# genetics-statistics/GEMMA

Hardware: AMD Instinct MI355X
Metric: SNPs/s (-lmm 1 Wald) at n=20k on 1/2/4/8 MI355X; U^T x HBM GB/s vs roofline (higher is better)
Workload: dtype f64 (U^T x as int8-digit MFMA products with exact int32 accumulation; every column of U scaled by its exact maximum and rounded to 6 base-256 digits = 2^-48 of that maximum -- fp64 keeps 2^-53 per entry; value_strict / strict_leg (7g6m: U^T x at or below the fp64 GEMM's own error) and fp64_gemm_path

## Files before the change

### gemma_amd/build.py

```python
import os
import shutil
import subprocess

HERE = os.path.dirname(os.path.abspath(__file__))
CSRC = os.path.join(HERE, "csrc")
LIB = os.path.join(HERE, "libgemma_hip.so")
UNITS = {
    "gemma_hip.hip": ["dgemm_mfma.hip.h", "lmm_grid.hip.h", "lmm_score_panel.hip.h", "i8gemm.hip.h", "i8gemm_sparse.hip.h", "i8gemm_sparse2.hip.h", "i8gemm_sparse2_r16.hip.h", "i8gemm_dense16.hip.h", "lmm_assoc.hip.h",
                      "lmm_search.hip.h", "comm.hip.h", "comm_shm.hpp", "kin_i8.hip.h", "ingest.hip.h", "qc.hip.h", "lm_assoc.hip.h", "mvlmm.hip.h",
                      "mvlmm_kernels.hip.h", "eigh_tu.h", "tu_common.h",
                      "abi_kinship.inc.h", "abi_eigen_qc.inc.h", "abi_lmm_stage.inc.h", "abi_utx.inc.h", "abi_lmm_batch.inc.h",
                      "abi_mvlmm.inc.h", "abi_gxe_lm.inc.h", "abi_kept_comm.inc.h", "abi_lmm_multi.inc.h", "abi_lmm_score_panel.inc.h", "abi_vc.inc.h", "vc_tu.h", "abi_prdt.inc.h", "prdt_tu.h",
                      "abi_mqs.inc.h", "mqs_tu.h", "abi_cor.inc.h", "cor_tu.h"],
    "eigh_tu.hip": ["dgemm_mfma.hip.h", "eigh.hip.h", "eigh2.hip.h", "eigh_tu.h", "tu_common.h"],
    "vc_tu.hip": ["dgemm_mfma.hip.h", "spd_inv.hip.h", "vc.hip.h", "vc_tu.h", "tu_common.h", "host_linalg.h", "../../include/gemma_vc_hybrid.hpp"],
    "prdt_tu.hip": ["dgemm_mfma.hip.h", "geno_mv.hip.h", "dev_common.hip.h", "eigh_tu.h", "prdt_tu.h", "tu_common.h", "spd_inv.hip.h", "prdt_mv.hip.h"],
    "mqs_tu.hip": ["dgemm_mfma.hip.h", "mqs.hip.h", "ci.hip.h", "dev_common.hip.h", "mqs_tu.h", "tu_common.h", "host_linalg.h"],
    "cor_tu.hip": ["dgemm_mfma.hip.h", "cor.hip.h", "dev_common.hip.h", "cor_tu.h", "tu_common.h"],
    "mvlmm_kernels.hip": ["mvlmm.hip.h", "mvlmm_kernels.hip.h"],
    "mvlmm_kernels_wide.hip": ["mvlmm.hip.h", "mvlmm_kernels.hip.h"],
    "mvlmm_kernels_rt.hip": ["mvlmm.hip.h", "mvlmm_kernels.hip.h"],
    "mvlmm_kernels_d6.hip": ["mvlmm.hip.h", "mvlmm_kernels.hip.h"],
    "mvlmm_kernels_d7.hip": ["mvlmm.hip.h", "mvlmm_kernels.hip.h"],
    "mvlmm_kernels_d8.hip": ["mvlmm.hip.h", "mvlmm_kernels.hip.h"],
}
PUBLIC_HEADER_USERS = ("gemma_hip.hip", "eigh_tu.hip", "vc_tu.hip", "prdt_tu.hip", "mqs_tu.hip", "cor_tu.hip")
SOURCES = list(UNITS)
HEADERS = sorted({h for hs in UNITS.values() for h in hs})


def hipcc():
    for cand in (os.environ.get("HIPCC"), "/opt/rocm/bin/hipcc", shutil.which("hipcc")):
        if cand and os.path.exists(cand):
            return cand
    raise RuntimeError("hipcc not found: the gfx950 library cannot be built")


def stale():
    if not os.path.exists(LIB):
        return True
    t = os.path.getmtime(LIB)
    deps = [os.path.join(CSRC, f) for f in SOURCES + HEADERS]
    deps.append(os.path.join(HERE, "..", "include", "gemma_hip.h"))
    return any(os.path.getmtime(d) > t for d in deps)


def build(force=False, verbose=False):
    if not force and not stale():
        return LIB
    cc = hipcc()
    objdir = os.path.join(HERE, "_obj")
    os.makedirs(objdir, exist_ok=True)
    procs, objs = [], []
    for src in SOURCES:
        obj = os.path.join(objdir, src.replace(".hip", ".o"))
        objs.append(obj)
        hdrs = UNITS[src]
        deps = [os.path.join(CSRC, f) for f in [src] + hdrs]
        if src in PUBLIC_HEADER_USERS:
            deps.append(os.path.join(HERE, "..", "include", "gemma_hip.h"))
        if not force and os.path.exists(obj) and all(os.path.getmtime(d) <= os.path.getmtime(obj) for d in deps):
            continue
        cmd = [cc, "--offload-arch=gfx950", "-O3", "-std=c++17", "-fPIC", "-c", os.path.join(CSRC, src), "-o", obj]
        if verbose:
            print(" ".join(cmd))
        procs.append((cmd, subprocess.Popen(cmd, cwd=CSRC)))
    for cmd, pr in procs:
        if pr.wait() != 0:
            raise subprocess.CalledProcessError(pr.returncode, cmd)
    cmd = [cc, "--offload-arch=gfx950", "-fPIC", "-shared", "-o", LIB] + objs
    if verbose:
        print(" ".join(cmd))
    subprocess.check_call(cmd, cwd=CSRC)
    return LIB


if __name__ == "__main__":
    print(build(force=True, verbose=True))
```

### gemma_amd/csrc/abi_lmm_batch.inc.h

```cpp

static void xp_release() {
  Ctx::XPipe &x = g_ctx.xp;
  if (x.P) (void)hipStreamDestroy(x.P);
  if (x.Q) (void)hipStreamDestroy(x.Q);
  if (x.in_ready) (void)hipEventDestroy(x.in_ready);
  if (x.ingest_done) (void)hipEventDestroy(x.ingest_done);
  x.ingest_done = nullptr;
  x.ingest_valid = false;
  for (int i = 0; i < 2; ++i) {
    if (x.prod_done[i]) (void)hipEventDestroy(x.prod_done[i]);
    if (x.post_done[i]) (void)hipEventDestroy(x.post_done[i]);
    x.prod_done[i] = x.post_done[i] = nullptr;
    x.post_valid[i] = false;
  }
  x.P = x.Q = nullptr;
  x.in_ready = nullptr;
  x.count = 0;
  x.pending = false;
  x.cus = -1;
  x.shadow_A.release(); x.shadow_C.release(); x.shadow_mean.release(); x.shadow_rowsur.release();
}
static int xp_init() {
  Ctx::XPipe &x = g_ctx.xp;
  const int ncu = g_ctx.prop.multiProcessorCount;
  int cus = g_ctx.knobs.pipe_cus;
  if (cus < 0 || cus * 2 > ncu || ncu % 32 != 0 || cus % 8 != 0 || (cus && (ncu / 8) % (cus / 8) != 0)) cus = 0;
  if (x.P && x.cus == cus) return GEMMA_HIP_OK;
  HIPCHK(hipDeviceSynchronize());
  xp_release();
  if (cus > 0) {
    const int words = ncu / 32, per_xcd = cus / 8, cu_per_xcd = ncu / 8, stepj = cu_per_xcd / per_xcd;
    std::vector<unsigned> mp((size_t)words, 0xFFFFFFFFu), mq((size_t)words, 0u);
    for (int j = 0; j < cu_per_xcd; j += stepj)
      for (int xcd = 0; xcd < 8; ++xcd) {
        const int c = 8 * j + xcd;
        mp[c >> 5] &= ~(1u << (c & 31));
        mq[c >> 5] |= 1u << (c & 31);
      }
    HIPCHK(hipExtStreamCreateWithCUMask(&x.P, (uint32_t)words, mp.data()));
    HIPCHK(hipExtStreamCreateWithCUMask(&x.Q, (uint32_t)words, mq.data()));
  } else {
    HIPCHK(hipStreamCreateWithFlags(&x.P, hipStreamDefault));
    HIPCHK(hipStreamCreateWithFlags(&x.Q, hipStreamDefault));
  }
  HIPCHK(hipEventCreateWithFlags(&x.in_ready, hipEventDisableTiming));
  HIPCHK(hipEventCreateWithFlags(&x.ingest_done, hipEventDisableTiming));
  for (int i = 0; i < 2; ++i) {
    HIPCHK(hipEventCreateWithFlags(&x.prod_done[i], hipEventDisableTiming));
    HIPCHK(hipEventCreateWithFlags(&x.post_done[i], hipEventDisableTiming));
  }
  x.cus = cus;
  return GEMMA_HIP_OK;
}
static int xp_flush(hipStream_t s) {
  Ctx::XPipe &x = g_ctx.xp;
  if (!x.pending) return GEMMA_HIP_OK;
  for (int i = 0; i < 2; ++i)
    if (x.post_valid[i]) HIPCHK(hipStreamWaitEvent(s, x.post_done[i], 0));
  x.pending = false;
  x.ingest_valid = false;
  return GEMMA_HIP_OK;
}
static int xp_abort(int rc) {
  Ctx::XPipe &x = g_ctx.xp;
  (void)hipDeviceSynchronize();
  x.count = 0;
  x.post_valid[0] = x.post_valid[1] = false;
  x.pending = false;
  x.ingest_valid = false;
  return rc;
}
static void xp_swap_sets() {
  Ctx::XPipe &x = g_ctx.xp;
  std::swap(g_ctx.i8_A, x.shadow_A); std::swap(g_ctx.i8_C, x.shadow_C);
  std::swap(g_ctx.i8_mean, x.shadow_mean); std::swap(g_ctx.i8_rowsur, x.shadow_rowsur);
}


static int compute_utx(int kind, const void *geno, size_t l, size_t ld, int path, double **UtX_out, size_t *ldx_out,
                       hipStream_t s) {
  {
    int rcf = xp_flush(s);
    if (rcf) return rcf;
  }
  const size_t n = g_ctx.cfg.n;
  const size_t ldx = (n + 1) & ~(size_t)1;
  const bool want_i8 = (path < 0 ? utx_i8_mode() == 1 : path == 1);
  const bool plink_i8 = want_i8 && kind == GEMMA_GENO_PLINK_2BIT;
  if (g_ctx.UtX.reserve(l * ldx * 8) || (!plink_i8 && g_ctx.X.reserve(l * ldx * 8)))
    return fail(GEMMA_HIP_ENOMEM, "lmm_batch: cannot allocate 2 x %zu bytes", l * ldx * 8);
  double *UtX = g_ctx.UtX.as<double>();
  *UtX_out = UtX;
  *ldx_out = ldx;
  g_ctx.last_utx_path = plink_i8 ? 1 : 0;
  if (plink_i8) return utx_plink_i8(geno, l, ld, UtX, ldx, s);
  double *X = g_ctx.X.as<double>();
  bool done = false;
  if (kind == GEMMA_GENO_F64_IDV_MAJOR) {
    {
      ProfScope ps(GEMMA_STAGE_INGEST, s);
      dim3 grid((unsigned)((l + 31) / 32), (unsigned)((n + 31) / 32));
      hipLaunchKernelGGL(transpose_kernel, grid, dim3(32, 8), 0, s, reinterpret_cast<const double *>(geno),
                         (long)n, (long)l, (long)ld, X, (long)ldx);
      HIPCHK(hipGetLastError());
    }
    if (want_i8) {
      int rc = utx_f64_try_i8(X, l, ldx, false, UtX, ldx, s, &done);
      if (rc) return rc;
    }
  } else if (kind == GEMMA_GENO_F64_SNP_MAJOR && want_i8) {
    int rc = utx_f64_try_i8(reinterpret_cast<const double *>(geno), l, ld, true, UtX, ldx, s, &done);
    if (rc) return rc;
  }
  if (done) return GEMMA_HIP_OK;
  if (kind != GEMMA_GENO_F64_IDV_MAJOR) {
    ProfScope ps(GEMMA_STAGE_INGEST, s);
    IngestArgs a;
    a.src = geno; a.ld = (long)ld; a.l = (long)l;
    a.idx_map = g_ctx.have_map ? g_ctx.idx_map.as<int>() : nullptr;
    a.n = (int)n; a.dst = X; a.ldo = (long)ldx; a.k_mode = 0;
    const unsigned grid = (unsigned)((l + 3) / 4);
    if (kind == GEMMA_GENO_PLINK_2BIT)
      hipLaunchKernelGGL(ingest_lmm_kernel<true>, dim3(grid), dim3(256), 0, s, a);
    else
      hipLaunchKernelGGL(ingest_lmm_kernel<false>, dim3(grid), dim3(256), 0, s, a);
    HIPCHK(hipGetLastError());
  }
  {
    ProfScope ps(GEMMA_STAGE_UTX_GEMM, s);
    const double *Ug;
    long ldu;
    int rcu = gemm_U(&Ug, &ldu, s);
    if (rcu) return rcu;
    note_utx_kernel(GEMMA_UTX_KERNEL_DGEMM_F64, 0, 0, 0);
    HIPCHK(launch_dgemm('N', 'N', (long)l, (long)n, (long)n, 1.0, X, (long)ldx, Ug, ldu, 0.0, UtX,
                        (long)ldx, false, false, s));
  }
  return GEMMA_HIP_OK;
}

static int check_batch_args(const char *who, int kind, const void *geno, size_t l, size_t ld, const void *out) {
  const size_t n = g_ctx.cfg.n;
  const size_t per_row = (kind == GEMMA_GENO_PLINK_2BIT && g_ctx.have_map) ? g_ctx.ni_total : n;
  const size_t need = min_ld_for(kind, per_row, l);
  if (need == (size_t)-1) return fail(GEMMA_HIP_EINVAL, "%s: unknown geno_kind %d", who, kind);
  if (!geno || !out || ld < need) return fail(GEMMA_HIP_EINVAL, "%s: ld=%zu < %zu", who, ld, need);
  return GEMMA_HIP_OK;
}

static int overlap_chunks(size_t l) {
  if (!g_ctx.knobs.overlap) return 1;
  if (utx_i8_mode() != 1 || i8_sparse_mode() != 2) return 1;
  int q = g_ctx.knobs.overlap_chunks;
  q = std::max(1, std::min(q, 16));
  while (q > 1 && l < (size_t)q * 2 * S2_BM) --q;
  return q;
}
static int overlap_init() {
  if (g_ctx.ov_stream) return GEMMA_HIP_OK;
  HIPCHK(hipStreamCreateWithFlags(&g_ctx.ov_stream, hipStreamNonBlocking));
  for (auto &e : g_ctx.ov_ready) HIPCHK(hipEventCreateWithFlags(&e, hipEventDisableTiming));
  HIPCHK(hipEventCreateWithFlags(&g_ctx.ov_done, hipEventDisableTiming));
  return GEMMA_HIP_OK;
}
static int lmm_batch_plink_chunked(const void *geno, size_t l, size_t ld, gemma_sumstat *out_d, int chunks, hipStream_t s) {
  const size_t n = g_ctx.cfg.n;
  const size_t ldx = (n + 1) & ~(size_t)1;
  int rc = overlap_init();
  if (rc) return rc;
  if (g_ctx.UtX.reserve(l * ldx * 8)) return fail(GEMMA_HIP_ENOMEM, "lmm_batch: cannot allocate %zu bytes", l * ldx * 8);
  double *UtX = g_ctx.UtX.as<double>();
  g_ctx.last_utx_path = 1;
  I8Dims d;
  if ((rc = i8_begin(l, &d, s))) return rc;
  {
    ProfScope ps(GEMMA_STAGE_INGEST, s);
    IngestI8Args a;
    a.src = reinterpret_cast<const unsigned char *>(geno); a.ld = (long)ld; a.l = (long)l;
    a.idx_map = g_ctx.have_map ? g_ctx.idx_map.as<int>() : nullptr;
    a.n = (int)d.n; a.A = g_ctx.i8_A.as<int8_t>(); a.ldk = (long)d.ldk;
    a.mean = g_ctx.i8_mean.as<double>();
    hipLaunchKernelGGL(ingest_i8_kernel, dim3((unsigned)((l + 3) / 4)), dim3(256), 0, s, a);
    HIPCHK(hipGetLastError());
  }
  if ((rc = i8_meta_build(d, s))) return rc;
  const size_t per = round_up((l + chunks - 1) / chunks, (size_t)S2_BM);
  hipStream_t side = g_ctx.ov_stream;
  int c = 0;
  for (size_t row0 = 0; row0 < l; row0 += per, ++c) {
    const size_t rows = std::min(per, l - row0), rows_pad = std::min(per, d.lpad - row0);
    if ((rc = i8_gemm_rows(d, row0, rows_pad, s, UtX, ldx, rows))) break;
    if (hipEventRecord(g_ctx.ov_ready[c], s) != hipSuccess || hipStreamWaitEvent(side, g_ctx.ov_ready[c], 0) != hipSuccess) {
      rc = fail(GEMMA_HIP_ERUNTIME, "lmm_batch: %s", hipGetErrorString(hipGetLastError()));
      break;
    }
    if ((rc = i8_post_rows(l, d, row0, rows, UtX, ldx, side))) break;
    if ((rc = launch_assoc(UtX + row0 * ldx, rows, ldx, out_d + row0, side))) break;
  }
  (void)hipEventRecord(g_ctx.ov_done, side);
  (void)hipStreamWaitEvent(s, g_ctx.ov_done, 0);
  return rc;
}

static int xp_flush_fwd(hipStream_t s) { return xp_flush(s); }

extern "C" int gemma_hip_lmm_pipe_flush(void *stream) {
  NEED_INIT();
  return xp_flush(S(stream));
}

extern "C" int gemma_hip_lmm_batch_pipe_d(int kind, const void *geno, size_t l, size_t ld, gemma_sumstat *out_d, void *stream) {
  NEED_INIT();
  if (!g_ctx.lmm_active) return fail(GEMMA_HIP_ESTATE, "lmm_batch_pipe before lmm_setup");
  NEED_SINGLE("lmm_batch_pipe");
  if (l == 0) return GEMMA_HIP_OK;
  int rc = check_batch_args("lmm_batch_pipe", kind, geno, l, ld, out_d);
  if (rc) return rc;
  hipStream_t s = S(stream);
  if (kind != GEMMA_GENO_PLINK_2BIT || utx_i8_mode() != 1 || i8_sparse_mode() != 2) {
    if ((rc = xp_flush(s))) return rc;
    return gemma_hip_lmm_batch_d(kind, geno, l, ld, out_d, stream);
  }
  if ((rc = xp_init())) return rc;
  Ctx::XPipe &x = g_ctx.xp;
  const int slot = (int)(x.count & 1);
  const size_t n = g_ctx.cfg.n;
  const size_t ldx = (n + 1) & ~(size_t)1;
  if (g_ctx.UtX.reserve(l * ldx * 8)) return fail(GEMMA_HIP_ENOMEM, "lmm_batch_pipe: cannot allocate %zu bytes", l * ldx * 8);
  if (s != nullptr && x.ingest_valid) HIPCHK(hipStreamWaitEvent(s, x.ingest_done, 0));
  xp_swap_sets();
  if (s != nullptr) {
    HIPCHK(hipEventRecord(x.in_ready, s));
    HIPCHK(hipStreamWaitEvent(x.P, x.in_ready, 0));
  }
  if (x.post_valid[slot]) HIPCHK(hipStreamWaitEvent(x.P, x.post_done[slot], 0));
  g_ctx.last_utx_path = 1;
  I8Dims d;
  if ((rc = i8_begin(l, &d, x.P, false))) return xp_abort(rc);
  {
    ProfScope ps(GEMMA_STAGE_INGEST, x.P);
    IngestI8Args a;
    a.src = reinterpret_cast<const unsigned char *>(geno); a.ld = (long)ld; a.l = (long)l;
    a.idx_map = g_ctx.have_map ? g_ctx.idx_map.as<int>() : nullptr;
    a.n = (int)d.n; a.A = g_ctx.i8_A.as<int8_t>(); a.ldk = (long)d.ldk;
    a.mean = g_ctx.i8_mean.as<double>();
    hipLaunchKernelGGL(ingest_i8_kernel, dim3((unsigned)((l + 3) / 4)), dim3(256), 0, x.P, a);
    if (hipGetLastError() != hipSuccess) return xp_abort(fail(GEMMA_HIP_ERUNTIME, "lmm_batch_pipe: ingest launch"));
  }
  if (hipEventRecord(x.ingest_done, x.P) != hipSuccess) return xp_abort(fail(GEMMA_HIP_ERUNTIME, "lmm_batch_pipe: event"));
  x.ingest_valid = true;
  if ((rc = i8_meta_build(d, x.P))) return xp_abort(rc);
  if ((rc = i8_gemm_rows(d, 0, d.lpad, x.P))) return xp_abort(rc);
  HIPCHK(hipEventRecord(x.prod_done[slot], x.P));
  HIPCHK(hipStreamWaitEvent(x.Q, x.prod_done[slot], 0));
  double *UtX = g_ctx.UtX.as<double>();
  rc = i8_post_rows(l, d, 0, l, UtX, ldx, x.Q);
  if (!rc) rc = launch_assoc(UtX, l, ldx, out_d, x.Q);
  (void)hipEventRecord(x.post_done[slot], x.Q);
  x.post_valid[slot] = true;
  x.pending = true;
  x.count += 1;
  return rc;
}

extern "C" int gemma_hip_lmm_batch_d(int kind, const void *geno, size_t l, size_t ld, gemma_sumstat *out_d,
                                     void *stream) {
  NEED_INIT();
  if (!g_ctx.lmm_active) return fail(GEMMA_HIP_ESTATE, "lmm_batch before lmm_setup");
  NEED_SINGLE("lmm_batch");
  if (l == 0) return GEMMA_HIP_OK;
  int rc = check_batch_args("lmm_batch", kind, geno, l, ld, out_d);
  if (rc) return rc;
  hipStream_t s = S(stream);
  if ((rc = xp_flush(s))) return rc;
  if (kind == GEMMA_GENO_PLINK_2BIT) {
    const int chunks = overlap_chunks(l);
    if (chunks > 1) return lmm_batch_plink_chunked(geno, l, ld, out_d, chunks, s);
  }
  double *UtX;
  size_t ldx;
  rc = compute_utx(kind, geno, l, ld, -1, &UtX, &ldx, s);
  if (rc) return rc;
  return launch_assoc(UtX, l, ldx, out_d, s);
}

extern "C" int gemma_hip_lmm_gene_batch_d(const double *Y_d, size_t l, size_t ld, gemma_sumstat *out_d, void *stream) {
  NEED_INIT();
  if (!g_ctx.lmm_active) return fail(GEMMA_HIP_ESTATE, "lmm_gene_batch before lmm_setup");
  NEED_SINGLE("lmm_gene_batch");
  if (l == 0) return GEMMA_HIP_OK;
  const size_t n = g_ctx.cfg.n, c = g_ctx.cfg.n_cvt;
  if (!Y_d || !out_d || ld < n) return fail(GEMMA_HIP_EINVAL, "lmm_gene_batch: ld=%zu < n=%zu", ld, n);
  hipStream_t s = S(stream);
  const size_t ldx = (n + 1) & ~(size_t)1;
  if (int rcf = xp_flush(S(stream))) return rcf;
  if (g_ctx.UtX.reserve(l * ldx * 8)) return fail(GEMMA_HIP_ENOMEM, "lmm_gene_batch: %zu bytes", l * ldx * 8);
  double *UtY = g_ctx.UtX.as<double>();
  {
    ProfScope ps(GEMMA_STAGE_UTX_GEMM, s);
    const double *Ug;
    long ldu;
    int rcu = gemm_U(&Ug, &ldu, s);
    if (rcu) return rcu;
    HIPCHK(launch_dgemm('N', 'N', (long)l, (long)n, (long)n, 1.0, Y_d, (long)ld, Ug, ldu, 0.0, UtY, (long)ldx,
                        false, false, s));
  }
  AssocArgs a = g_ctx.assoc_proto;
  a.UtX = UtY; a.ld = (long)ldx; a.l = (long)l;
  a.eval = g_ctx.eval; a.Uty = g_ctx.Uty; a.UtWt = g_ctx.UtWt.as<double>();
  a.out = reinterpret_cast<SumStat *>(out_d);
  a.grid_T = nullptr;
  a.have_grid = 0;
  const unsigned grid = (unsigned)((l + 3) / 4);
  {
    ProfScope ps(GEMMA_STAGE_ASSOC, s);
    switch (c) {
    case 1: hipLaunchKernelGGL(lmm_gene_kernel<1>, dim3(grid), dim3(256), 0, s, a); break;
    case 2: hipLaunchKernelGGL(lmm_gene_kernel<2>, dim3(grid), dim3(256), 0, s, a); break;
    case 3: hipLaunchKernelGGL(lmm_gene_kernel<3>, dim3(grid), dim3(256), 0, s, a); break;
    case 4: hipLaunchKernelGGL(lmm_gene_kernel<4>, dim3(grid), dim3(256), 0, s, a); break;
    default:
      if (c > (size_t)GEN_CMAX) {
        int rcw = wide_attr(lmm_gene_wide_kernel);
        if (rcw) return rcw;
        hipLaunchKernelGGL(lmm_gene_wide_kernel, dim3((unsigned)l), dim3(64), wide_lds_bytes(c), s, a, (int)c);
      } else {
        hipLaunchKernelGGL(lmm_gene_generic_kernel, dim3(grid), dim3(256), 0, s, a, (int)c);
      }
      break;
    }
    HIPCHK(hipGetLastError());
  }
  return GEMMA_HIP_OK;
}

extern "C" int gemma_hip_lmm_gene_batch(const double *Y, size_t l, size_t ld, gemma_sumstat *out) {
  NEED_INIT();
  if (!g_ctx.lmm_active) return fail(GEMMA_HIP_ESTATE, "lmm_gene_batch before lmm_setup");
  NEED_SINGLE("lmm_gene_batch");
  if (l == 0) return GEMMA_HIP_OK;
  const size_t n = g_ctx.cfg.n;
  if (!Y || !out || ld < n) return fail(GEMMA_HIP_EINVAL, "lmm_gene_batch: ld=%zu < n=%zu", ld, n);
  if (g_ctx.stage_in.reserve(l * ld * 8) || g_ctx.stage_out.reserve(l * sizeof(gemma_sumstat)))
    return fail(GEMMA_HIP_ENOMEM, "lmm_gene_batch: staging %zu bytes", l * ld * 8);
  HIPCHK(hipMemcpy(g_ctx.stage_in.p, Y, l * ld * 8, hipMemcpyHostToDevice));
  int rc = gemma_hip_lmm_gene_batch_d(g_ctx.stage_in.as<double>(), l, ld, g_ctx.stage_out.as<gemma_sumstat>(), nullptr);
  if (rc) return rc;
  HIPCHK(hipMemcpy(out, g_ctx.stage_out.p, l * sizeof(gemma_sumstat), hipMemcpyDeviceToHost));
  return GEMMA_HIP_OK;
}
```

### gemma_amd/csrc/abi_utx.inc.h

```cpp

struct I8Dims {
  size_t n, ldk, npad, lpad, mrows;
  int fuse, digits, nplanes;
  int mdrop;
  int complete;
  int epi;
};
static const int *i8_anymiss(const I8Dims &d) { return d.complete ? g_ctx.i8_rowsur.as<int>() + d.lpad : nullptr; }
static int i8_sparse_mode() { return g_ctx.knobs.i8_sparse; }
static int i8_begin(size_t l, I8Dims *d, hipStream_t s, bool allow_epi = true) {
  int rc = i8_prepare_u(s);
  if (rc) return rc;
  d->n = g_ctx.cfg.n; d->ldk = g_ctx.i8_ldk; d->npad = g_ctx.i8_npad;
  d->lpad = round_up(l, i8_sparse_mode() == 2 ? (size_t)S2_BM : (size_t)I8P_BM); d->mrows = 2 * d->lpad;
  d->fuse = (g_ctx.knobs.i8_fuse && (double)d->n * 2.0 * 128.0 * 257.0 < 2147483648.0) ? 1 : 0;
  d->digits = g_ctx.i8_digits;
  d->nplanes = d->fuse ? (d->digits + 1) / 2 : d->digits;
  d->mdrop = (g_ctx.knobs.i8_mdrop && d->fuse && d->digits == 7 && i8_sparse_mode() == 2 && g_ctx.knobs.i8_rows == 16) ? 1 : 0;
  d->complete = (g_ctx.knobs.i8_complete && i8_sparse_mode() == 2 && g_ctx.knobs.i8_rows == 16) ? 1 : 0;
  d->epi = (allow_epi && g_ctx.knobs.i8_epilogue && i8_sparse_mode() == 2 && g_ctx.knobs.i8_rows == 16 && d->nplanes >= 2) ? 1 : 0;
  const size_t c_elems = (size_t)(d->nplanes - d->epi) * d->mrows * d->npad;
  if (g_ctx.i8_A.reserve(d->lpad * d->ldk) || g_ctx.i8_C.reserve(c_elems * 4) || g_ctx.i8_mean.reserve(l * 8))
    return fail(GEMMA_HIP_ENOMEM, "lmm_batch: int8 product buffers (%zu bytes)", d->lpad * d->ldk + c_elems * 4);
  if (d->lpad != l) HIPCHK(hipMemsetAsync(g_ctx.i8_A.p, 0, d->lpad * d->ldk, s));
  return GEMMA_HIP_OK;
}

static int i8_meta_build(const I8Dims &d, hipStream_t s) {
  const int mode = i8_sparse_mode();
  if (mode == 0) return GEMMA_HIP_OK;
  ProfScope ps(GEMMA_STAGE_INGEST, s);
  const size_t nk = d.ldk / I8_BK, total = d.lpad * nk * (mode == 2 ? 4 : 2);
  if (g_ctx.i8_meta.reserve(total * sizeof(uint4)) || g_ctx.i8_rowsur.reserve((d.lpad + 1) * sizeof(int)))
    return fail(GEMMA_HIP_ENOMEM, "lmm_batch: mask words of the sparse product");
  HIPCHK(hipMemsetAsync(g_ctx.i8_rowsur.p, 0, (d.lpad + 1) * sizeof(int), s));
  if (mode == 2)
    hipLaunchKernelGGL(sparse2_meta_kernel, dim3((unsigned)((total + 255) / 256)), dim3(256), 0, s, g_ctx.i8_A.as<int8_t>(),
                       (long)d.lpad, (long)d.ldk, g_ctx.i8_meta.as<uint4>(), g_ctx.i8_rowsur.as<int>(),
                       const_cast<int *>(i8_anymiss(d)));
  else
    hipLaunchKernelGGL(sparse_meta_kernel, dim3((unsigned)((total + 255) / 256)), dim3(256), 0, s, g_ctx.i8_A.as<int8_t>(),
                       (long)d.lpad, (long)d.ldk, g_ctx.i8_meta.as<uint4>(), g_ctx.i8_rowsur.as<int>());
  HIPCHK(hipGetLastError());
  g_ctx.i8_flag_at = (mode == 2 && d.complete) ? (long)d.lpad : -1;
  g_ctx.i8_rowsur_n = (long)d.lpad;
  return GEMMA_HIP_OK;
}

static int raster_for(int tiles_m, int tiles_n, int rb, hipStream_t s, const int2 **map_d) {
  Ctx::RasterSlot *lru = &g_ctx.i8_raster[0];
  for (auto &r : g_ctx.i8_raster) {
    if (r.tm == tiles_m && r.tn == tiles_n && r.rb == rb && r.dev.p) {
      r.used = ++g_ctx.i8_raster_clock;
      *map_d = r.dev.as<int2>();
      return GEMMA_HIP_OK;
    }
    if (r.used < lru->used) lru = &r;
  }
  if (lru->dev.p) HIPCHK(hipDeviceSynchronize());
  s2_build_raster(tiles_m, tiles_n, rb, lru->host);
  lru->tm = lru->tn = lru->rb = 0;
  if (lru->dev.reserve(lru->host.size() * sizeof(int2)))
    return fail(GEMMA_HIP_ENOMEM, "lmm_batch: tile raster (%zu bytes)", lru->host.size() * sizeof(int2));
  HIPCHK(hipMemcpyAsync(lru->dev.p, lru->host.data(), lru->host.size() * sizeof(int2), hipMemcpyHostToDevice, s));
  HIPCHK(hipStreamSynchronize(s));
  lru->tm = tiles_m; lru->tn = tiles_n; lru->rb = rb;
  lru->used = ++g_ctx.i8_raster_clock;
  *map_d = lru->dev.as<int2>();
  return GEMMA_HIP_OK;
}

static int i8_gemm_rows(const I8Dims &d, size_t row0, size_t rows_pad, hipStream_t s, double *UtX = nullptr, size_t ldx = 0,
                        size_t rows = 0) {
  const int mode = i8_sparse_mode();
  const bool sparse = mode != 0;
  if (d.epi && (mode != 2 || g_ctx.knobs.i8_rows != 16 || !UtX || rows == 0))
    return fail(GEMMA_HIP_ESTATE, "lmm_batch: the epilogue form of the int8 product without its destination");
  g_ctx.i8_last_epi = d.epi;
  ProfScope ps(GEMMA_STAGE_UTX_GEMM, s);
  static bool attr_set = false;
  if (!attr_set) {
    HIPCHK(hipFuncSetAttribute(reinterpret_cast<const void *>(i8gemm_packed_kernel_t<true>),
                               hipFuncAttributeMaxDynamicSharedMemorySize, 3 * I8P_STAGE));
    attr_set = true;
  }
  I8PackArgs g;
  g.A = g_ctx.i8_A.as<int8_t>();
  g.Bt = g_ctx.i8_Bt.as<int8_t>();
  g.C = g_ctx.i8_C.as<int>();
  g.ldk = (long)d.ldk; g.ldc = (long)d.npad;
  g.strideB = (long)(d.npad * d.ldk); g.strideC = (long)(d.mrows * d.npad);
  g.m_row0 = (long)d.lpad;
  g.tiles_m = (int)(d.lpad / I8P_BM); g.tiles_n = (int)(d.npad / I8_BN);
  g.nk = (int)(d.ldk / I8_BK);
  g.gm = g_ctx.knobs.i8_gm;
  g.fuse = d.fuse;
  g.digits = d.digits;
  const dim3 grid((unsigned)(g.tiles_m * g.tiles_n), (unsigned)d.nplanes);
  if (mode == 2) {
    static bool attr3 = false;
    if (!attr3) {
      HIPCHK(hipFuncSetAttribute(reinterpret_cast<const void *>(i8gemm_sparse2_kernel),
                                 hipFuncAttributeMaxDynamicSharedMemorySize, S2_NST * S2_STAGE));
      HIPCHK(hipFuncSetAttribute(reinterpret_cast<const void *>(i8gemm_sparse2_r16_kernel),
                                 hipFuncAttributeMaxDynamicSharedMemorySize, S2_R16_LDS));
      HIPCHK(hipFuncSetAttribute(reinterpret_cast<const void *>(i8gemm_sparse2_r16_g_kernel),
                                 hipFuncAttributeMaxDynamicSharedMemorySize, S2_R16_LDS));
      HIPCHK(hipFuncSetAttribute(reinterpret_cast<const void *>(i8gemm_sparse2_r16_ep_kernel),
                                 hipFuncAttributeMaxDynamicSharedMemorySize, S2_R16_LDS));
      HIPCHK(hipFuncSetAttribute(reinterpret_cast<const void *>(i8gemm_sparse2_r16_ep_g_kernel),
                                 hipFuncAttributeMaxDynamicSharedMemorySize, S2_R16_LDS));
      attr3 = true;
    }
    Sparse2Args g2;
    g2.AM = g_ctx.i8_meta.as<uint4>() + (row0 / S2_BM) * (size_t)g.nk * S2_BM * 4;
    g2.Bt = g.Bt; g2.C = g.C + row0 * (size_t)g.ldc - (d.epi ? g.strideC : 0); g2.ldk = g.ldk; g2.ldc = g.ldc; g2.strideB = g.strideB; g2.strideC = g.strideC;
    g2.m_row0 = g.m_row0;
    g2.tiles_m = (int)(rows_pad / S2_BM); g2.tiles_n = (int)(d.npad / S2_BN);
    g2.nk = g.nk; g2.gm = g.gm; g2.fuse = g.fuse; g2.digits = g.digits;
    int raster_rb = 0;
    {
      const int rb = g_ctx.knobs.i8_raster;
      if (rb > 0) {
        const int2 *map_d = nullptr;
        int rc_map = raster_for(g2.tiles_m, g2.tiles_n, rb, s, &map_d);
        if (rc_map) return rc_map;
        g2.tile_map = map_d;
        raster_rb = rb;
      }
    }
    note_utx_kernel(g_ctx.knobs.i8_rows == 32 ? GEMMA_UTX_KERNEL_RECORDS_R32 : GEMMA_UTX_KERNEL_RECORDS_R16, d.digits, d.fuse,
                    raster_rb);
    if (g_ctx.knobs.i8_rows == 32) {
      hipLaunchKernelGGL(i8gemm_sparse2_kernel, dim3((unsigned)(g2.tiles_m * g2.tiles_n), (unsigned)d.nplanes), dim3(512),
                         S2_NST * S2_STAGE, s, g2);
    } else if (d.epi) {
      const unsigned wgs = (unsigned)(g2.tiles_m * g2.tiles_n);
      g2.anymiss = i8_anymiss(d);
      g2.plane0 = 1;
      g2.run_if = g2.anymiss ? 1 : 0;
      hipLaunchKernelGGL(i8gemm_sparse2_r16_kernel, dim3(wgs, (unsigned)d.nplanes - 1u), dim3(512), S2_R16_LDS, s, g2);
      if (g2.anymiss) {
        g2.run_if = 2;
        hipLaunchKernelGGL(i8gemm_sparse2_r16_g_kernel, dim3(wgs, (unsigned)d.nplanes - 1u), dim3(512), S2_R16_LDS, s, g2);
      }
      g2.plane0 = 0;
      g2.UtX = UtX + row0 * ldx; g2.ldx = (long)ldx; g2.l = (long)rows; g2.n = (long)d.n;
      g2.mean = g_ctx.i8_mean.as<double>() + row0; g2.qinv = g_ctx.i8_qinv.as<double>();
      g2.m_scale = 1.0; g2.nplanes = d.nplanes;
      if (d.mdrop) {
        g2.run_if = 0;
        hipLaunchKernelGGL(i8gemm_sparse2_r16_ep_g_kernel, dim3(wgs, 1u), dim3(512), S2_R16_LDS, s, g2);
      } else {
        g2.run_if = g2.anymiss ? 1 : 0;
        hipLaunchKernelGGL(i8gemm_sparse2_r16_ep_kernel, dim3(wgs, 1u), dim3(512), S2_R16_LDS, s, g2);
        if (g2.anymiss) {
          g2.run_if = 2;
          hipLaunchKernelGGL(i8gemm_sparse2_r16_ep_g_kernel, dim3(wgs, 1u), dim3(512), S2_R16_LDS, s, g2);
        }
      }
    } else {
      const unsigned wgs = (unsigned)(g2.tiles_m * g2.tiles_n), first = d.mdrop ? 1u : 0u;
      g2.anymiss = i8_anymiss(d);
      g2.plane0 = (int)first;
      g2.run_if = g2.anymiss ? 1 : 0;
      hipLaunchKernelGGL(i8gemm_sparse2_r16_kernel, dim3(wgs, (unsigned)d.nplanes - first), dim3(512), S2_R16_LDS, s, g2);
      if (g2.anymiss) {
        g2.run_if = 2;
        hipLaunchKernelGGL(i8gemm_sparse2_r16_g_kernel, dim3(wgs, (unsigned)d.nplanes - first), dim3(512), S2_R16_LDS, s, g2);
      }
      if (d.mdrop) {
        g2.plane0 = 0; g2.run_if = 0;
        hipLaunchKernelGGL(i8gemm_sparse2_r16_g_kernel, dim3(wgs, 1u), dim3(512), S2_R16_LDS, s, g2);
      }
    }
  } else if (sparse) {
    static bool attr2 = false;
    if (!attr2) {
      HIPCHK(hipFuncSetAttribute(reinterpret_cast<const void *>(i8gemm_sparse_kernel),
                                 hipFuncAttributeMaxDynamicSharedMemorySize, 3 * SP_STAGE));
      attr2 = true;
    }
    SparseMeta sm;
    sm.m4 = g_ctx.i8_meta.as<uint4>();
    sm.row_surplus = g_ctx.i8_rowsur.as<int>();
    sm.ntiles = (long)g.nk;
    note_utx_kernel(GEMMA_UTX_KERNEL_SPARSE_BYTES, d.digits, d.fuse, 0);
    hipLaunchKernelGGL(i8gemm_sparse_kernel, grid, dim3(512), 3 * SP_STAGE, s, g, sm);
  } else {
    note_utx_kernel(GEMMA_UTX_KERNEL_DENSE_I8, d.digits, d.fuse, 0);
    hipLaunchKernelGGL(i8gemm_packed_kernel_t<true>, grid, dim3(512), 3 * I8P_STAGE, s, g);
  }
  HIPCHK(hipGetLastError());
  return GEMMA_HIP_OK;
}

static int i8_post_rows(size_t l, const I8Dims &d, size_t row0, size_t rows, double *UtX, size_t ldx, hipStream_t s) {
  const bool sparse = i8_sparse_mode() != 0;
  ProfScope ps(GEMMA_STAGE_UTX_POST, s);
  int *sur_cnt = nullptr, *sur_list = nullptr;
  const int8_t *Arow = g_ctx.i8_A.as<int8_t>() + row0 * d.ldk;
  if (sparse) {
    if (g_ctx.i8_surlist.reserve(l * (SUR_MAX + 1) * sizeof(int)))
      return fail(GEMMA_HIP_ENOMEM, "lmm_batch: dropped-call lists");
    sur_cnt = g_ctx.i8_surlist.as<int>() + row0;
    sur_list = g_ctx.i8_surlist.as<int>() + l + row0 * SUR_MAX;
    hipLaunchKernelGGL(i8_surplus_list_kernel, dim3((unsigned)((rows + 3) / 4)), dim3(256), 0, s, Arow, (long)d.ldk,
                       g_ctx.i8_rowsur.as<int>() + row0, (long)rows, sur_cnt, sur_list);
    HIPCHK(hipGetLastError());
  }
  if (!d.epi) {
    hipLaunchKernelGGL(i8_combine_kernel, dim3((unsigned)((d.n + 1023) / 1024), (unsigned)std::min<size_t>(rows, 65535)),
                       dim3(256), 0, s,
                       g_ctx.i8_C.as<int>() + row0 * d.npad, (long)d.npad, (long)(d.mrows * d.npad), (long)d.lpad,
                       g_ctx.i8_mean.as<double>() + row0, g_ctx.i8_qinv.as<double>(), (long)rows, (long)d.n, UtX + row0 * ldx, (long)ldx,
                       1.0, d.fuse, d.digits, sur_cnt, sur_list, g_ctx.U, (long)d.n, d.mdrop, i8_anymiss(d));
    HIPCHK(hipGetLastError());
  } else if (sparse) {
    hipLaunchKernelGGL(i8_surplus_short_kernel, dim3((unsigned)rows), dim3(256), 0, s, sur_cnt, sur_list,
                       g_ctx.i8_mean.as<double>() + row0, g_ctx.U, (long)d.n, (long)d.n, (long)rows, UtX + row0 * ldx, (long)ldx);
    HIPCHK(hipGetLastError());
  }
  if (sparse) {
    hipLaunchKernelGGL(i8_surplus_fix_kernel, dim3((unsigned)rows), dim3(256), 0, s, Arow, (long)d.ldk,
                       g_ctx.i8_rowsur.as<int>() + row0, g_ctx.i8_mean.as<double>() + row0, g_ctx.U, (long)d.n, (long)d.n,
                       (long)rows, UtX + row0 * ldx, (long)ldx, SUR_MAX);
    HIPCHK(hipGetLastError());
  }
  return GEMMA_HIP_OK;
}

static int i8_product(size_t l, const I8Dims &d, double *UtX, size_t ldx, hipStream_t s) {
  int rc = i8_meta_build(d, s);
  if (!rc) rc = i8_gemm_rows(d, 0, d.lpad, s, UtX, ldx, l);
  if (!rc) rc = i8_post_rows(l, d, 0, l, UtX, ldx, s);
  return rc;
}

static int utx_plink_i8(const void *geno, size_t l, size_t ld, double *UtX, size_t ldx, hipStream_t s) {
  I8Dims d;
  int rc = i8_begin(l, &d, s);
  if (rc) return rc;
  {
    ProfScope ps(GEMMA_STAGE_INGEST, s);
    IngestI8Args a;
    a.src = reinterpret_cast<const unsigned char *>(geno); a.ld = (long)ld; a.l = (long)l;
    a.idx_map = g_ctx.have_map ? g_ctx.idx_map.as<int>() : nullptr;
    a.n = (int)d.n; a.A = g_ctx.i8_A.as<int8_t>(); a.ldk = (long)d.ldk;
    a.mean = g_ctx.i8_mean.as<double>();
    hipLaunchKernelGGL(ingest_i8_kernel, dim3((unsigned)((l + 3) / 4)), dim3(256), 0, s, a);
    HIPCHK(hipGetLastError());
  }
  return i8_product(l, d, UtX, ldx, s);
}

static bool dosage_i8_enabled() { return g_ctx.knobs.dosage_i8 != 0; }
static int utx_dosage_i8(const double *src, size_t l, size_t ld, bool nan_missing, bool two, bool have_m, const I8Dims &d,
                         double *UtX, size_t ldx, hipStream_t s) {
  const int np = (two ? 2 : 1) + (have_m ? 1 : 0);
  const size_t plane_a = d.lpad * d.ldk, plane_c = d.lpad * d.npad;
  if (g_ctx.i8_A.reserve((size_t)np * plane_a) || g_ctx.i8_C.reserve((size_t)np * d.digits * plane_c * 4) ||
      g_ctx.i8_colsum.reserve(d.n * 8))
    return fail(GEMMA_HIP_ENOMEM, "lmm_batch: dosage planes (%zu bytes)", (size_t)np * (plane_a + d.digits * plane_c * 4));
  int8_t *A0 = g_ctx.i8_A.as<int8_t>();
  {
    ProfScope ps(GEMMA_STAGE_INGEST, s);
    if (d.lpad != l) HIPCHK(hipMemsetAsync(A0, 0, (size_t)np * plane_a, s));
    PackDosageArgs a;
    a.src = src; a.ld = (long)ld; a.l = (long)l; a.n = (int)d.n; a.nan_missing = nan_missing ? 1 : 0; a.two = two ? 1 : 0;
    a.A0 = A0; a.A1 = two ? A0 + plane_a : nullptr; a.Am = have_m ? A0 + (size_t)(np - 1) * plane_a : nullptr;
    a.ldk = (long)d.ldk; a.mean = g_ctx.i8_mean.as<double>();
    hipLaunchKernelGGL(pack_dosage_kernel, dim3((unsigned)((l + 3) / 4)), dim3(256), 0, s, a);
    HIPCHK(hipGetLastError());
    if (!g_ctx.i8_colsum_ready) {
      hipLaunchKernelGGL(u_digit_colsum_kernel, dim3((unsigned)((d.n + 3) / 4)), dim3(256), 0, s, g_ctx.i8_Bt.as<int8_t>(),
                         (long)d.ldk, (long)(d.npad * d.ldk), g_ctx.i8_qinv.as<double>(), (long)d.n, d.digits,
                         g_ctx.i8_colsum.as<double>());
      HIPCHK(hipGetLastError());
      g_ctx.i8_colsum_ready = true;
    }
  }
  {
    ProfScope ps(GEMMA_STAGE_UTX_GEMM, s);
    static bool attr_set = false;
    if (!attr_set) {
      HIPCHK(hipFuncSetAttribute(reinterpret_cast<const void *>(i8gemm_packed_kernel_t<false, true>),
                                 hipFuncAttributeMaxDynamicSharedMemorySize, 3 * I8P_STAGE));
      HIPCHK(hipFuncSetAttribute(reinterpret_cast<const void *>(i8gemm_dense16_kernel_t<true>),
                                 hipFuncAttributeMaxDynamicSharedMemorySize, 3 * I8P_STAGE));
      attr_set = true;
    }
    for (int a = 0; a < np; ++a) {
      I8PackArgs g;
      g.A = A0 + (size_t)a * plane_a;
      g.Bt = g_ctx.i8_Bt.as<int8_t>();
      g.C = g_ctx.i8_C.as<int>() + (size_t)a * d.digits * plane_c;
      g.ldk = (long)d.ldk; g.ldc = (long)d.npad;
      g.strideB = (long)(d.npad * d.ldk); g.strideC = (long)plane_c;
      g.m_row0 = 0;
      g.tiles_m = (int)(d.lpad / I8P_BM); g.tiles_n = (int)(d.npad / I8_BN);
      g.nk = (int)(d.ldk / I8_BK);
      g.gm = g_ctx.knobs.i8_gm;
      g.fuse = 0;
      g.digits = d.digits;
      if (g_ctx.knobs.dosage_rows == 32) {
        note_utx_kernel(GEMMA_UTX_KERNEL_DOSAGE_I8, d.digits, 0, 0);
        hipLaunchKernelGGL((i8gemm_packed_kernel_t<false, true>), dim3((unsigned)(g.tiles_m * g.tiles_n), (unsigned)d.digits),
                           dim3(512), 3 * I8P_STAGE, s, g);
      } else {
        note_utx_kernel(GEMMA_UTX_KERNEL_DOSAGE_I8_R16, d.digits, 0, 0);
        hipLaunchKernelGGL((i8gemm_dense16_kernel_t<true>), dim3((unsigned)(g.tiles_m * g.tiles_n), (unsigned)d.digits),
                           dim3(512), 3 * I8P_STAGE, s, g);
      }
      HIPCHK(hipGetLastError());
    }
  }
  {
    ProfScope ps(GEMMA_STAGE_UTX_POST, s);
    hipLaunchKernelGGL(i8_combine_dosage_kernel, dim3((unsigned)((d.n + 255) / 256), (unsigned)std::min<size_t>(l, 65535)),
                       dim3(256), 0, s, g_ctx.i8_C.as<int>(), (long)d.npad, (long)plane_c, g_ctx.i8_mean.as<double>(),
                       g_ctx.i8_qinv.as<double>(), g_ctx.i8_colsum.as<double>(), (long)l, (long)d.n, UtX, (long)ldx, d.digits,
                       two ? 1 : 0, have_m ? 1 : 0, two ? 1000.0 : 100.0);
    HIPCHK(hipGetLastError());
  }
  return GEMMA_HIP_OK;
}

static int utx_f64_try_i8(const double *src, size_t l, size_t ld, bool nan_missing, double *UtX, size_t ldx,
                          hipStream_t s, bool *done) {
  *done = false;
  I8Dims d;
  int rc = i8_begin(l, &d, s);
  if (rc) return rc;
  if (g_ctx.scratch.reserve(16)) return fail(GEMMA_HIP_ENOMEM, "lmm_batch: scratch");
  const int init[4] = {1, 1, 1, 0};
  HIPCHK(hipMemcpyAsync(g_ctx.scratch.p, init, sizeof init, hipMemcpyHostToDevice, s));
  {
    ProfScope ps(GEMMA_STAGE_INGEST, s);
    PackF64Args a;
    a.src = src; a.ld = (long)ld; a.l = (long)l; a.n = (int)d.n; a.nan_missing = nan_missing ? 1 : 0;
    a.A = g_ctx.i8_A.as<int8_t>(); a.ldk = (long)d.ldk; a.mean = g_ctx.i8_mean.as<double>();
    a.all_hard = g_ctx.scratch.as<int>();
    hipLaunchKernelGGL(pack_f64_kernel, dim3((unsigned)((l + 3) / 4)), dim3(256), 0, s, a);
    HIPCHK(hipGetLastError());
  }
  int verdict[4] = {0, 0, 0, 0};
  HIPCHK(hipMemcpyAsync(verdict, g_ctx.scratch.p, sizeof verdict, hipMemcpyDeviceToHost, s));
  HIPCHK(hipStreamSynchronize(s));
  if (verdict[0]) {
    *done = true;
    g_ctx.last_utx_path = 1;
    return i8_product(l, d, UtX, ldx, s);
  }
  if (verdict[1] && dosage_i8_enabled()) {
    *done = true;
    g_ctx.last_utx_path = verdict[2] ? 2 : 3;
    return utx_dosage_i8(src, l, ld, nan_missing, !verdict[2], verdict[3] != 0, d, UtX, ldx, s);
  }
  return GEMMA_HIP_OK;
}

static int gemm_U(const double **U, long *ld, hipStream_t s) {
  const size_t n = g_ctx.cfg.n;
  *U = g_ctx.U;
  *ld = (long)n;
  if ((n & 1) == 0) return GEMMA_HIP_OK;
  if (g_ctx.U_even_of != g_ctx.U) {
    if (g_ctx.U_even.reserve(n * (n + 1) * 8)) return fail(GEMMA_HIP_ENOMEM, "lmm_batch: even-ld copy of U");
    HIPCHK(hipMemcpy2DAsync(g_ctx.U_even.p, (n + 1) * 8, g_ctx.U, n * 8, n * 8, n, hipMemcpyDeviceToDevice, s));
    g_ctx.U_even_of = g_ctx.U;
  }
  *U = g_ctx.U_even.as<double>();
  *ld = (long)n + 1;
  return GEMMA_HIP_OK;
}
```

### gemma_amd/csrc/gemma_hip.hip

```cpp
#include <hip/hip_runtime.h>

#include <cmath>
#include <cstdarg>
#include <cstdio>
#include <cstdlib>
#include <cstring>
#include <string>
#include <vector>

#include "../../include/gemma_hip.h"
#include "tu_common.h"
#include "dgemm_mfma.hip.h"
#include "eigh_tu.h"
#include "vc_tu.h"
#include "prdt_tu.h"
#include "mqs_tu.h"
#include "cor_tu.h"
#include "ingest.hip.h"
#include "lm_assoc.hip.h"
#include "lmm_assoc.hip.h"
#include "lmm_grid.hip.h"
#include "lmm_score_panel.hip.h"
#include "i8gemm.hip.h"
#include "i8gemm_sparse.hip.h"
#include "i8gemm_sparse2.hip.h"
#include "i8gemm_sparse2_r16.hip.h"
#include "i8gemm_dense16.hip.h"
#include "qc.hip.h"
#include "mvlmm.hip.h"
#include "comm.hip.h"
#include "kin_i8.hip.h"

using namespace gemma_hip;

namespace {

struct StageProf {
  std::vector<std::pair<hipEvent_t, hipEvent_t>> ev;
  double acc_ms = 0.0;
  long launches = 0;
};

struct Knobs {
  int utx_i8 = 1;
  int i8_digits = 0;
  int i8_sparse = 2;
  int i8_fuse = 1;
  int i8_gm = 0;
  int i8_raster = S2_DEFAULT_RASTER;
  int i8_rows = 16;
  int i8_scale_max = 1;
  int i8_mdrop = 0;
  int i8_complete = 1;
  int i8_epilogue = 1;
  int dosage_i8 = 1;
  int dosage_rows = 16;
  int overlap = 0;
  int overlap_chunks = 4;
  int table_v2 = 1;
  int table_pf = 0;
  int multi_table = 1;
  int force_generic = 0;
  int assoc_variant = 44;
  int mvlmm_rt = 0;
  int pipe_cus = 64;
  int kin_i8 = 1, kin_upper = 1, kin_lists = 1, kin_lists_oom = 0;
  long long kin_list_cap = 0;
  static int geti(const char *name, int dflt) {
    const char *e = getenv(name);
    return (e && *e) ? atoi(e) : dflt;
  }
  void load() {
    utx_i8 = geti("GEMMA_HIP_UTX_I8", 1);
    const int dg = geti("GEMMA_HIP_I8_DIGITS", 0);
    i8_digits = (dg == 6 || dg == 7) ? dg : 0;
    const char *es = getenv("GEMMA_HIP_I8_SPARSE");
    i8_sparse = (es && es[0] >= '0' && es[0] <= '2') ? es[0] - '0' : 2;
    const char *ef = getenv("GEMMA_HIP_I8_FUSE");
    i8_fuse = (ef && ef[0] == '0') ? 0 : 1;
    i8_gm = geti("GEMMA_HIP_I8_GM", 0);
    i8_raster = geti("GEMMA_HIP_I8_RASTER", S2_DEFAULT_RASTER);
    i8_rows = geti("GEMMA_HIP_I8_ROWS", 16) == 32 ? 32 : 16;
    const char *esc = getenv("GEMMA_HIP_I8_SCALE");
    i8_scale_max = (esc && strcmp(esc, "pow2") == 0) ? 0 : 1;
    const char *efm = getenv("GEMMA_HIP_I8_FORM");
    i8_mdrop = (efm && strcmp(efm, "7g6m") == 0) ? 1 : 0;
    if (i8_mdrop) i8_digits = 7;
    const char *ecp = getenv("GEMMA_HIP_I8_COMPLETE");
    i8_complete = (ecp && ecp[0] == '0') ? 0 : 1;
    const char *eep = getenv("GEMMA_HIP_I8_EPILOGUE");
    i8_epilogue = (eep && eep[0] == '0') ? 0 : 1;
    const char *ed = getenv("GEMMA_HIP_UTX_DOSAGE_I8");
    dosage_i8 = (ed && ed[0] == '0') ? 0 : 1;
    dosage_rows = geti("GEMMA_HIP_DOSAGE_ROWS", 16) == 32 ? 32 : 16;
    const char *eo = getenv("GEMMA_HIP_OVERLAP");
    overlap = (eo && eo[0] == '1') ? 1 : 0;
    overlap_chunks = geti("GEMMA_HIP_OVERLAP_CHUNKS", 4);
    const char *et = getenv("GEMMA_HIP_TABLE_V2");
    table_v2 = (et && et[0] == '0') ? 0 : 1;
    const char *ep = getenv("GEMMA_HIP_TABLE_PF");
    table_pf = (ep && ep[0] == '1') ? 1 : 0;
    const char *em = getenv("GEMMA_HIP_MULTI_TABLE");
    multi_table = (em && em[0] == '0') ? 0 : 1;
    const char *eg = getenv("GEMMA_HIP_FORCE_GENERIC");
    force_generic = (eg && eg[0] == '1') ? 1 : 0;
    assoc_variant = geti("GEMMA_HIP_ASSOC_VARIANT", 44);
    const char *er = getenv("GEMMA_HIP_MVLMM_RT");
    mvlmm_rt = (er && er[0] == '1') ? 1 : 0;
    pipe_cus = geti("GEMMA_HIP_PIPE_CUS", 64);
    const char *k1 = getenv("GEMMA_HIP_KIN_I8"), *k2 = getenv("GEMMA_HIP_KIN_UPPER"), *k3 = getenv("GEMMA_HIP_KIN_LISTS");
    const char *k4 = getenv("GEMMA_HIP_KIN_LISTS_OOM"), *k5 = getenv("GEMMA_HIP_KIN_LIST_CAP");
    kin_i8 = (k1 && k1[0] == '0') ? 0 : 1;
    kin_upper = (k2 && k2[0] == '0') ? 0 : 1;
    kin_lists = (k3 && k3[0] == '0') ? 0 : 1;
    kin_lists_oom = (k4 && k4[0] == '1') ? 1 : 0;
    kin_list_cap = (k5 && *k5) ? atoll(k5) : 0;
  }
};

struct Ctx {
  bool inited = false;
  Knobs knobs;
  int device = -1;
  int verbose = 0;
  std::string last_error;
  hipDeviceProp_t prop;
  bool profiling = false;
  StageProf prof[GEMMA_STAGE_COUNT];

  bool kin_active = false;
  size_t kin_n = 0;
  int kin_mode = 1;
  size_t kin_ns = 0;
  DevBuf kin_K, kin_X, kin_stage;
  hipStream_t kin_copy = nullptr;
  hipEvent_t kin_copied = nullptr, kin_ingested = nullptr;
  bool kin_ingested_valid = false, kin_host_call = false;
  DevBuf qc_G, qc_M, qc_W, qc_O;
  bool kin_i8 = false, kin_i8_used = false;
  DevBuf i8_meta, i8_rowsur;
  DevBuf U_even;
  const double *U_even_of = nullptr;
  DevBuf kin_GtG, kin_S, kin_a, kin_At, kin_Gt;
  DevBuf kin_A2, kin_cnt, kin_off, kin_listS, kin_listJ, kin_sub, kin_cj, kin_flag;
  DevBuf kin_tmap;
  hipStream_t ov_stream = nullptr;
  hipEvent_t ov_ready[16] = {}, ov_done = nullptr;
  struct XPipe {
    hipStream_t P = nullptr, Q = nullptr;
    hipEvent_t in_ready = nullptr, prod_done[2] = {}, post_done[2] = {};
    hipEvent_t ingest_done = nullptr;
    bool ingest_valid = false;
    bool post_valid[2] = {false, false};
    unsigned long long count = 0;
    bool pending = false;
    int cus = -1;
    DevBuf shadow_A, shadow_C, shadow_mean, shadow_rowsur;
  } xp;
  int kin_tmap_tm = 0, kin_tmap_tn = 0, kin_tmap_count = 0;

  bool lmm_active = false;
  gemma_lmm_cfg cfg;
  const double *U = nullptr, *eval = nullptr, *Uty = nullptr;
  DevBuf own_U, own_eval, own_Uty, own_UtW, UtWt, idx_map;
  size_t ni_total = 0;
  bool have_map = false;
  DevBuf X, UtX, stage_in, stage_out, carry;
  DevBuf grid_R, grid_F, grid_T;
  DevBuf cheb_R, cheb_F, cheb_T, cheb_slots, cheb_list, cheb_count, cheb_D, cheb_Ck, cheb_Gk, cheb_Lk, cheb_iv, cheb_dends, cheb_res;
  double cheb_mid[ASSOC_MAX_REGION], cheb_inv_half[ASSOC_MAX_REGION];
  GridGeom cheb_geom;
  DevBuf table_P;
  DevBuf gxe_env, gxe_UtWt, gxe_Z, gxe_UtZ, gxe_flip;
  bool gxe_ready = false;
  double gxe_lnbeta = 0.0;
  DevBuf mv_Yt, mv_out;
  DevBuf mv_scratch;
  bool mv_ready = false, mv_gxe = false;
  size_t mv_d = 0;
  MvArgs mv_proto;
  DevBuf i8_Bt, i8_q, i8_qinv, i8_cmax, i8_A, i8_C, i8_mean;
  unsigned long long cheb_qmask = 0;
  struct RasterSlot {
    DevBuf dev;
    std::vector<int2> host;
    int tm = 0, tn = 0, rb = 0, xcds = 8;
    unsigned long long used = 0;
  } i8_raster[6];
  unsigned long long i8_raster_clock = 0;
  DevBuf i8_surlist;
  DevBuf i8_colsum;
  bool i8_colsum_ready = false;
  int last_utx_path = 0;
  gemma_utx_kernel_info last_utx_kernel = {};
  int i8_last_epi = -1;
  long i8_rowsur_n = 0;
  long i8_flag_at = -1;
  bool i8_ready = false;
  size_t i8_ldk = 0, i8_npad = 0;
  int i8_digits = I8_DIGITS;
  GridGeom grid_geom;
  int carry_flip = 0;
  AssocArgs assoc_proto;
  struct PhenoSlot {
    AssocArgs proto;
    const double *Uty = nullptr;
    DevBuf grid_R, grid_F, cheb_R, cheb_F, carry;
    GridGeom grid_geom, cheb_geom;
    double cheb_mid[ASSOC_MAX_REGION], cheb_inv_half[ASSOC_MAX_REGION];
    unsigned long long cheb_qmask = 0;
    int carry_flip = 0;
  };
  std::vector<PhenoSlot> slots;
  size_t multi_T = 0;
  DevBuf multi_Yt;
  DevBuf multi_R, multi_T_buf;
  int multi_G = 0;
  size_t score_T = 0;
  ScoreGeom score_geom;
  DevBuf score_R, score_Pyy, score_Yt, score_lam, score_bad;
  DevBuf score_fthr, score_cells, score_hits, score_cnt, score_best;
  double score_fthr_p = -1.0;
  hipStream_t score_fthr_s = nullptr;

  bool lm_active = false;
  LmArgs lm_proto;
  DevBuf lm_Wt, lm_y, lm_small;

  DevBuf scratch;

  struct PipeSlot {
    void *pin_in = nullptr, *pin_out = nullptr;
    size_t pin_in_cap = 0, pin_out_cap = 0;
    DevBuf dev_in, dev_out;
    hipEvent_t h2d = nullptr, done = nullptr;
    size_t l = 0;
    bool busy = false;
  } pipe[2];
  hipStream_t pipe_copy = nullptr, pipe_comp = nullptr;
  int pipe_head = 0, pipe_count = 0;

  DevBuf kept_K, kept_UE;
  size_t kept_K_n = 0, kept_n = 0;
  double kept_trace = 0.0;
  Comm comm;
} g_ctx;

int fail(int code, const char *fmt, ...) {
  char buf[512];
  va_list ap;
  va_start(ap, fmt);
  vsnprintf(buf, sizeof buf, fmt, ap);
  va_end(ap);
  g_ctx.last_error = buf;
  if (g_ctx.verbose) fprintf(stderr, "gemma_hip: %s\n", buf);
  return code;
}

int ret(int rc, const std::string &msg) { return rc ? fail(rc, "%s", msg.c_str()) : GEMMA_HIP_OK; }

#define HIPCHK(expr)                                                                        \
  do {                                                                                      \
    hipError_t e_ = (expr);                                                                 \
    if (e_ != hipSuccess)                                                                   \
      return fail(GEMMA_HIP_ERUNTIME, "%s failed: %s (%s:%d)", #expr, hipGetErrorString(e_), \
                  __FILE__, __LINE__);                                                      \
  } while (0)

#define NEED_INIT()                                                                              \
  do {                                                                                           \
    if (!g_ctx.inited) {                                                                         \
      int rc_ = gemma_hip_init(-1, 0);                                                           \
      if (rc_ != GEMMA_HIP_OK) return rc_;                                                       \
    }                                                                                            \
  } while (0)

struct ProfScope {
  int stage;
  hipStream_t s;
  hipEvent_t a = nullptr, b = nullptr;
  ProfScope(int st, hipStream_t stream) : stage(st), s(stream) {
    if (g_ctx.profiling) {
      if (hipEventCreate(&a) == hipSuccess && hipEventCreate(&b) == hipSuccess)
        (void)hipEventRecord(a, s);
      else
        a = b = nullptr;
    }
  }
  ~ProfScope() {
    if (a && b) {
      (void)hipEventRecord(b, s);
      g_ctx.prof[stage].ev.emplace_back(a, b);
    }
  }
};

int prof_collect(int stage) {
  StageProf &p = g_ctx.prof[stage];
  for (auto &pr : p.ev) {
    (void)hipEventSynchronize(pr.second);
    float ms = 0.f;
    if (hipEventElapsedTime(&ms, pr.first, pr.second) == hipSuccess) {
      p.acc_ms += ms;
      p.launches += 1;
    }
    (void)hipEventDestroy(pr.first);
    (void)hipEventDestroy(pr.second);
  }
  p.ev.clear();
  return GEMMA_HIP_OK;
}

inline hipStream_t S(void *s) { return reinterpret_cast<hipStream_t>(s); }

}

static void pipe_release();
static void xp_release();
static int xp_flush_fwd(hipStream_t s);
static void raster_release() {
  for (auto &r : g_ctx.i8_raster) {
    r.dev.release();
    r.host.clear();
    r.tm = r.tn = r.rb = 0;
    r.used = 0;
  }
}
static void kin_i8_release();

extern "C" int gemma_hip_abi_version(void) { return GEMMA_HIP_ABI_VERSION; }

extern "C" const char *gemma_hip_strerror(int code) {
  switch (code) {
  case GEMMA_HIP_OK: return "ok";
  case GEMMA_HIP_EINVAL: return "invalid argument (range error)";
  case GEMMA_HIP_ENODEV: return "no usable gfx950 device";
  case GEMMA_HIP_ENOMEM: return "device memory allocation failed";
  case GEMMA_HIP_ERUNTIME: return "HIP runtime error";
  case GEMMA_HIP_ESTATE: return "call sequence violated";
  case GEMMA_HIP_ENOCONV: return "eigensolver did not converge";
  case GEMMA_HIP_ENOTPD: return "matrix not positive definite";
  default: return "unknown error";
  }
}

extern "C" const char *gemma_hip_last_error(void) { return g_ctx.last_error.c_str(); }

extern "C" int gemma_hip_init(int device, int verbose) {
  g_ctx.verbose = verbose;
  int ndev = 0;
  if (hipGetDeviceCount(&ndev) != hipSuccess || ndev <= 0) {
    (void)hipGetLastError();
    return fail(GEMMA_HIP_ENODEV, "no HIP device visible (this library has no CPU fallback)");
  }
  if (device >= 0) {
    if (device >= ndev) return fail(GEMMA_HIP_ENODEV, "device %d out of range (%d visible)", device, ndev);
    HIPCHK(hipSetDevice(device));
  }
  int cur = 0;
  HIPCHK(hipGetDevice(&cur));
  HIPCHK(hipGetDeviceProperties(&g_ctx.prop, cur));
  if (strncmp(g_ctx.prop.gcnArchName, "gfx950", 6) != 0)
    return fail(GEMMA_HIP_ENODEV, "device %d is %s; this build targets gfx950 only", cur,
                g_ctx.prop.gcnArchName);
  g_ctx.device = cur;
  g_ctx.inited = true;
  g_ctx.knobs.load();
  gemm_aux_init();
  if (verbose)
    fprintf(stderr, "gemma_hip: device %d %s (%s), %d CUs, %.1f GB\n", cur, g_ctx.prop.name,
            g_ctx.prop.gcnArchName, g_ctx.prop.multiProcessorCount,
            (double)g_ctx.prop.totalGlobalMem / 1e9);
  return GEMMA_HIP_OK;
}

extern "C" void gemma_hip_shutdown(void) {
  if (!g_ctx.inited) return;
  (void)hipDeviceSynchronize();
  for (int s = 0; s < GEMMA_STAGE_COUNT; ++s) prof_collect(s);
  g_ctx.kin_K.release(); g_ctx.kin_X.release(); g_ctx.kin_stage.release();
  g_ctx.qc_G.release(); g_ctx.qc_M.release(); g_ctx.qc_W.release(); g_ctx.qc_O.release();
  kin_i8_release();
  g_ctx.own_U.release(); g_ctx.own_eval.release(); g_ctx.own_Uty.release(); g_ctx.own_UtW.release();
  g_ctx.UtWt.release(); g_ctx.idx_map.release(); g_ctx.X.release(); g_ctx.UtX.release();
  g_ctx.stage_in.release(); g_ctx.stage_out.release(); g_ctx.carry.release(); g_ctx.scratch.release();
  g_ctx.i8_Bt.release(); g_ctx.i8_q.release(); g_ctx.i8_qinv.release(); g_ctx.i8_cmax.release(); g_ctx.i8_A.release(); g_ctx.i8_C.release();
  raster_release();
  g_ctx.mv_Yt.release(); g_ctx.mv_out.release(); g_ctx.mv_scratch.release();
  g_ctx.mv_ready = g_ctx.mv_gxe = false;
  g_ctx.i8_mean.release(); g_ctx.i8_meta.release(); g_ctx.i8_rowsur.release(); g_ctx.i8_colsum.release(); g_ctx.i8_surlist.release();
  g_ctx.i8_ready = g_ctx.i8_colsum_ready = false;
  g_ctx.table_P.release(); g_ctx.U_even.release();
  for (auto &p : g_ctx.slots) { p.grid_R.release(); p.grid_F.release(); p.cheb_R.release(); p.cheb_F.release(); p.carry.release(); }
  g_ctx.slots.clear();
  g_ctx.multi_Yt.release(); g_ctx.multi_R.release(); g_ctx.multi_T_buf.release();
  g_ctx.multi_T = 0;
  g_ctx.score_R.release(); g_ctx.score_Pyy.release(); g_ctx.score_Yt.release(); g_ctx.score_lam.release(); g_ctx.score_bad.release();
  g_ctx.score_fthr.release(); g_ctx.score_cells.release(); g_ctx.score_hits.release(); g_ctx.score_cnt.release(); g_ctx.score_best.release();
  g_ctx.score_fthr_p = -1.0;
  g_ctx.score_T = 0;
  g_ctx.U_even_of = nullptr;
  pipe_release();
  xp_release();
  if (g_ctx.ov_stream) {
    (void)hipStreamDestroy(g_ctx.ov_stream);
    for (auto &e : g_ctx.ov_ready)
      if (e) (void)hipEventDestroy(e);
    if (g_ctx.ov_done) (void)hipEventDestroy(g_ctx.ov_done);
    g_ctx.ov_stream = nullptr;
    for (auto &e : g_ctx.ov_ready) e = nullptr;
    g_ctx.ov_done = nullptr;
  }
  if (g_ctx.kin_copy) {
    (void)hipStreamDestroy(g_ctx.kin_copy);
    if (g_ctx.kin_copied) (void)hipEventDestroy(g_ctx.kin_copied);
    if (g_ctx.kin_ingested) (void)hipEventDestroy(g_ctx.kin_ingested);
    g_ctx.kin_copy = nullptr;
    g_ctx.kin_copied = g_ctx.kin_ingested = nullptr;
    g_ctx.kin_ingested_valid = false;
  }
  g_ctx.kin_active = g_ctx.lmm_active = false;
  g_ctx.kept_K.release(); g_ctx.kept_UE.release();
  g_ctx.kept_K_n = g_ctx.kept_n = 0;
  g_ctx.comm.finalize();
  gemm_aux_destroy();
  eigh_tu_shutdown();
  vc_tu_shutdown();
  prdt_tu_shutdown();
  mqs_tu_shutdown();
  cor_tu_shutdown();
  g_ctx.inited = false;
}

extern "C" int gemma_hip_device_info(char *name, size_t len, int *n_cu, size_t *hbm_bytes) {
  NEED_INIT();
  if (name && len) {
    snprintf(name, len, "%s (%s)", g_ctx.prop.name, g_ctx.prop.gcnArchName);
  }
  if (n_cu) *n_cu = g_ctx.prop.multiProcessorCount;
  if (hbm_bytes) *hbm_bytes = g_ctx.prop.totalGlobalMem;
  return GEMMA_HIP_OK;
}

extern "C" int gemma_hip_profile_enable(int on) {
  g_ctx.profiling = (on != 0);
  return GEMMA_HIP_OK;
}

extern "C" int gemma_hip_profile_read(int stage, double *total_ms, long *launches, int reset) {
  NEED_INIT();
  if (stage < 0 || stage >= GEMMA_STAGE_COUNT) return fail(GEMMA_HIP_EINVAL, "bad stage %d", stage);
  prof_collect(stage);
  if (total_ms) *total_ms = g_ctx.prof[stage].acc_ms;
  if (launches) *launches = g_ctx.prof[stage].launches;
  if (reset) {
    g_ctx.prof[stage].acc_ms = 0.0;
    g_ctx.prof[stage].launches = 0;
  }
  return GEMMA_HIP_OK;
}

static int check_gemm(char ta, char tb, size_t M, size_t N, size_t K, size_t lda, size_t ldb,
                      size_t ldc) {
  const bool tA = (ta == 'T' || ta == 't'), tB = (tb == 'T' || tb == 't');
  if (!tA && ta != 'N' && ta != 'n') return fail(GEMMA_HIP_EINVAL, "dgemm: bad TransA '%c'", ta);
  if (!tB && tb != 'N' && tb != 'n') return fail(GEMMA_HIP_EINVAL, "dgemm: bad TransB '%c'", tb);
  const size_t a_cols = tA ? M : K, b_cols = tB ? K : N;
  if (lda < a_cols || ldb < b_cols || ldc < N)
    return fail(GEMMA_HIP_EINVAL, "Range error in dgemm (lda=%zu ldb=%zu ldc=%zu for M=%zu N=%zu K=%zu)",
                lda, ldb, ldc, M, N, K);
  return GEMMA_HIP_OK;
}

extern "C" int gemma_hip_dgemm_d(char ta, char tb, size_t M, size_t N, size_t K, double alpha,
                                 const double *A, size_t lda, const double *B, size_t ldb,
                                 double beta, double *C, size_t ldc, void *stream) {
  NEED_INIT();
  int rc = check_gemm(ta, tb, M, N, K, lda, ldb, ldc);
  if (rc) return rc;
  if (M == 0 || N == 0) return GEMMA_HIP_OK;
  ProfScope ps(GEMMA_STAGE_UTX_GEMM, S(stream));
  HIPCHK(launch_dgemm(ta, tb, (long)M, (long)N, (long)K, alpha, A, (long)lda, B, (long)ldb, beta, C,
                      (long)ldc, false, false, S(stream)));
  return GEMMA_HIP_OK;
}

extern "C" int gemma_hip_dgemm(char ta, char tb, size_t M, size_t N, size_t K, double alpha,
                               const double *A, size_t lda, const double *B, size_t ldb,
                               double beta, double *C, size_t ldc) {
  NEED_INIT();
  int rc = check_gemm(ta, tb, M, N, K, lda, ldb, ldc);
  if (rc) return rc;
  if (M == 0 || N == 0) return GEMMA_HIP_OK;
  const bool tA = (ta == 'T' || ta == 't'), tB = (tb == 'T' || tb == 't');
  const size_t a_rows = tA ? K : M, b_rows = tB ? N : K;
  const size_t a_bytes = a_rows * lda * 8, b_bytes = b_rows * ldb * 8, c_bytes = M * ldc * 8;
  DevBuf dA, dB, dC;
  if (dA.reserve(a_bytes ? a_bytes : 8) || dB.reserve(b_bytes ? b_bytes : 8) || dC.reserve(c_bytes)) {
    dA.release(); dB.release(); dC.release();
    return fail(GEMMA_HIP_ENOMEM, "dgemm: cannot allocate %zu bytes", a_bytes + b_bytes + c_bytes);
  }
  auto h2d = [&](void *d, const double *h, size_t rows, size_t cols, size_t ld) -> hipError_t {
    if (rows == 0 || cols == 0) return hipSuccess;
    return hipMemcpy2D(d, ld * 8, h, ld * 8, cols * 8, rows, hipMemcpyHostToDevice);
  };
  hipError_t e = h2d(dA.p, A, a_rows, tA ? M : K, lda);
  if (e == hipSuccess) e = h2d(dB.p, B, b_rows, tB ? K : N, ldb);
  if (e == hipSuccess && beta != 0.0) e = h2d(dC.p, C, M, N, ldc);
  if (e == hipSuccess)
    e = launch_dgemm(ta, tb, (long)M, (long)N, (long)K, alpha, dA.as<double>(), (long)lda,
                     dB.as<double>(), (long)ldb, beta, dC.as<double>(), (long)ldc, false, false, 0);
  if (e == hipSuccess) e = hipMemcpy2D(C, ldc * 8, dC.p, ldc * 8, N * 8, M, hipMemcpyDeviceToHost);
  dA.release(); dB.release(); dC.release();
  if (e != hipSuccess) return fail(GEMMA_HIP_ERUNTIME, "dgemm: %s", hipGetErrorString(e));
  return GEMMA_HIP_OK;
}

#include "abi_kinship.inc.h"
#include "abi_eigen_qc.inc.h"
#include "abi_lmm_stage.inc.h"
#include "abi_utx.inc.h"
#include "abi_lmm_batch.inc.h"
#include "abi_mvlmm.inc.h"
#include "abi_gxe_lm.inc.h"
#include "abi_kept_comm.inc.h"
#include "abi_lmm_multi.inc.h"
#include "abi_lmm_score_panel.inc.h"
#include "abi_vc.inc.h"
#include "abi_prdt.inc.h"
#include "abi_mqs.inc.h"
#include "abi_cor.inc.h"
```

### gemma_amd/csrc/i8gemm_sparse.hip.h

```cpp
#pragma once
#include "i8gemm.hip.h"

namespace gemma_hip {

typedef int i32x8 __attribute__((ext_vector_type(8)));
constexpr int SP_STAGE = I8P_STAGE + 4096;

struct SparseMeta {
  const uint4 *m4;
  int *row_surplus;
  long ntiles;
};

__global__ __launch_bounds__(256) void sparse_meta_kernel(const int8_t *__restrict__ A, long lpad, long ldk, uint4 *__restrict__ m4,
                                                          int *__restrict__ row_surplus) {
  const long nk = ldk / I8_BK;
  const long id = (long)blockIdx.x * 256 + threadIdx.x;
  if (id >= lpad * nk * 2) return;
  const long row = id / (nk * 2), rem = id % (nk * 2), tile = rem >> 1;
  const int h = (int)(rem & 1);
  unsigned w[4];
  int surplus = 0;
#pragma unroll
  for (int p = 0; p < 2; ++p) {
    const int8_t *src = A + row * ldk + tile * I8_BK + 32 * (2 * p + h);
    unsigned idx = 0, bits = 0;
    for (int gq = 0; gq < 8; ++gq) {
      const unsigned word = *reinterpret_cast<const unsigned *>(src + 4 * gq);
      const unsigned m = (word >> 4) & 0x01010101u;
      const unsigned pat = (m | (m >> 7) | (m >> 14) | (m >> 21)) & 0xFu;
      const int cnt = __popc(pat);
      const int p0 = cnt >= 1 ? __ffs(pat) - 1 : 0;
      const unsigned rest = pat & (pat - 1);
      const int p1 = cnt >= 2 ? __ffs(rest) - 1 : (p0 == 3 ? 2 : 3);
      idx |= (unsigned)(p0 | (p1 << 2)) << (4 * gq);
      bits |= (unsigned)((cnt >= 1) | ((cnt >= 2) << 1)) << (2 * gq);
      surplus += cnt > 2 ? cnt - 2 : 0;
    }
    w[2 * p] = idx;
    w[2 * p + 1] = bits;
  }
  m4[id] = make_uint4(w[0], w[1], w[2], w[3]);
  if (surplus) atomicAdd(row_surplus + row, surplus);
}

static inline int sparse_meta_build(const int8_t *A, long lpad, long ldk, SparseMeta *sm) {
  const long nk = ldk / I8_BK, total = lpad * nk * 2;
  uint4 *m4 = nullptr;
  int *rs = nullptr;
  if (hipMalloc(reinterpret_cast<void **>(&m4), (size_t)total * sizeof(uint4)) != hipSuccess ||
      hipMalloc(reinterpret_cast<void **>(&rs), (size_t)lpad * sizeof(int)) != hipSuccess)
    return 1;
  (void)hipMemset(rs, 0, (size_t)lpad * sizeof(int));
  hipLaunchKernelGGL(sparse_meta_kernel, dim3((unsigned)((total + 255) / 256)), dim3(256), 0, 0, A, lpad, ldk, m4, rs);
  sm->m4 = m4;
  sm->row_surplus = rs;
  sm->ntiles = nk;
  return hipGetLastError() == hipSuccess ? 0 : 1;
}

__global__ __launch_bounds__(256) void i8_surplus_fix_kernel(const int8_t *__restrict__ A, long ldk,
                                                             const int *__restrict__ row_surplus,
                                                             const double *__restrict__ mean, const double *__restrict__ U,
                                                             long ldu, long n, long l, double *__restrict__ UtX, long ldx,
                                                             int skip_upto) {
  const long s = blockIdx.x;
  if (s >= l || row_surplus[s] <= skip_upto) return;
  __shared__ int found[256][2], list[512], nlist;
  const int t = threadIdx.x;
  const double mu = mean[s];
  const long ngroups = ldk / 4;
  for (long g0 = 0; g0 < ngroups; g0 += 256) {
    const long gq = g0 + t;
    int f0 = -1, f1 = -1;
    if (gq < ngroups) {
      const unsigned word = *reinterpret_cast<const unsigned *>(A + s * ldk + 4 * gq);
      const unsigned m = (word >> 4) & 0x01010101u;
      unsigned pat = (m | (m >> 7) | (m >> 14) | (m >> 21)) & 0xFu;
      if (__popc(pat) > 2) {
        pat &= pat - 1;
        pat &= pat - 1;
        f0 = (int)(4 * gq) + __ffs(pat) - 1;
        pat &= pat - 1;
        if (pat) f1 = (int)(4 * gq) + __ffs(pat) - 1;
      }
    }
    if (!__syncthreads_or(f0 >= 0)) continue;
    found[t][0] = f0;
    found[t][1] = f1;
    __syncthreads();
    if (t == 0) {
      int c = 0;
      for (int q = 0; q < 256; ++q)
        for (int e = 0; e < 2; ++e)
          if (found[q][e] >= 0) list[c++] = found[q][e];
      nlist = c;
    }
    __syncthreads();
    const int c = nlist;
    for (long k = t; k < n; k += 256) {
      double acc = 0.0;
      for (int e = 0; e < c; ++e) acc += U[(long)list[e] * ldu + k];
      UtX[s * ldx + k] += mu * acc;
    }
    __syncthreads();
  }
}

static_assert(SUR_MAX >= 2, "SUR_MAX (i8gemm.hip.h) is the list stride of this kernel, of i8_combine_kernel and of the host's buffers");
__global__ __launch_bounds__(256) void i8_surplus_list_kernel(const int8_t *__restrict__ A, long ldk, const int *__restrict__ row_surplus,
                                                             long l, int *__restrict__ sur_cnt, int *__restrict__ sur_list) {
  const int lane = threadIdx.x & 63;
  const long s = (long)blockIdx.x * 4 + (threadIdx.x >> 6);
  if (s >= l) return;
  const int want = row_surplus[s];
  if (want == 0 || want > SUR_MAX) {
    if (lane == 0) sur_cnt[s] = want == 0 ? 0 : -1;
    return;
  }
  int have = 0;
  const long ngroups = ldk / 4;
  for (long g0 = 0; g0 < ngroups && have < want; g0 += 64) {
    const long gq = g0 + lane;
    int f0 = -1, f1 = -1;
    if (gq < ngroups) {
      const unsigned word = *reinterpret_cast<const unsigned *>(A + s * ldk + 4 * gq);
      const unsigned m = (word >> 4) & 0x01010101u;
      unsigned pat = (m | (m >> 7) | (m >> 14) | (m >> 21)) & 0xFu;
      if (__popc(pat) > 2) {
        pat &= pat - 1;
        pat &= pat - 1;
        f0 = (int)(4 * gq) + __ffs(pat) - 1;
        pat &= pat - 1;
        if (pat) f1 = (int)(4 * gq) + __ffs(pat) - 1;
      }
    }
    const int mine = (f0 >= 0) + (f1 >= 0);
    int before = mine;
    for (int o = 1; o < 64; o <<= 1) {
      const int v = __shfl_up(before, o, 64);
      if (lane >= o) before += v;
    }
    const int base = have + before - mine;
    if (f0 >= 0) sur_list[s * SUR_MAX + base] = f0;
    if (f1 >= 0) sur_list[s * SUR_MAX + base + 1] = f1;
    have += __shfl(before, 63, 64);
  }
  if (lane == 0) sur_cnt[s] = have;
}

__global__ __launch_bounds__(256) void i8_surplus_short_kernel(const int *__restrict__ sur_cnt, const int *__restrict__ sur_list,
                                                               const double *__restrict__ mean, const double *__restrict__ U,
                                                               long ldu, long n, long l, double *__restrict__ UtX, long ldx) {
  const long s = blockIdx.x;
  if (s >= l) return;
  const int cnt = sur_cnt[s];
  if (cnt <= 0) return;
  const double mu = mean[s];
  for (long k = threadIdx.x; k < n; k += 256) {
    double acc = 0.0;
    for (int e = 0; e < cnt; ++e) acc += U[(long)sur_list[s * SUR_MAX + e] * ldu + k];
    double v = UtX[s * ldx + k];
    v += mu * acc;
    UtX[s * ldx + k] = v;
  }
}

__device__ __forceinline__ i32x4 sp_expand(unsigned bits) {
  i32x4 v;
#pragma unroll
  for (int d = 0; d < 4; ++d) v[d] = (int)((((bits >> (4 * d)) & 0xFu) * 0x00204081u) & 0x01010101u);
  return v;
}

__global__ __launch_bounds__(512, 2) void i8gemm_sparse_kernel(I8PackArgs g, SparseMeta sm) {
  extern __shared__ __attribute__((aligned(1024))) int8_t i8lds[];
  int tm, tn;
  {
    const int nwg = gridDim.x, b = blockIdx.x;
    const int q = nwg >> 3, r = nwg & 7, x = b & 7, o = b >> 3;
    const int L = (x < r ? x * (q + 1) : r * (q + 1) + (x - r) * q) + o;
    const int GM = g.gm > 0 ? g.gm : 8;
    const int per_group = GM * g.tiles_n;
    const int grp = L / per_group;
    const int first_m = grp * GM;
    const int gsz = min(g.tiles_m - first_m, GM);
    const int in = L - grp * per_group;
    tm = first_m + in % gsz;
    tn = in / gsz;
  }
  const int plane = blockIdx.y;
  const int odd = g.digits & 1;
  const int d_first = g.fuse ? (odd ? (plane == 0 ? 0 : 2 * plane) : 2 * plane + 1) : plane;
  const int nd = (g.fuse && !(odd && plane == 0)) ? 2 : 1;
  const int t = threadIdx.x, lane = t & 63;
  const int wave = __builtin_amdgcn_readfirstlane(t >> 6);
  const int wm = wave >> 2, wn = wave & 3;
  const int r32 = lane & 31, h = lane >> 5;

  const int8_t *src[6];
  int dst[6];
#define SP_INIT_SRC(DIGIT)                                                                                        \
  do {                                                                                                            \
    _Pragma("unroll") for (int j = 0; j < 6; ++j) {                                                               \
      const int p = 6 * wave + j;                                                                                 \
      const bool isA = p < 16;                                                                                    \
      const int row = 8 * (isA ? p : p - 16) + (lane >> 3);                                                       \
      const int chunk = (lane & 7) ^ ((row >> 1) & 7);                                                            \
      const int8_t *base = isA ? g.A + ((long)tm * I8P_BM + row) * g.ldk                                          \
                               : g.Bt + (long)(DIGIT) * g.strideB + ((long)tn * I8_BN + row) * g.ldk;             \
      src[j] = base + 16 * chunk;                                                                                 \
      dst[j] = p * 1024;                                                                                          \
    }                                                                                                             \
  } while (0)
  int fa[4], fb[4];
#pragma unroll
  for (int ks = 0; ks < 4; ++ks) {
    const int sw = ((2 * ks + h) ^ ((r32 >> 1) & 7)) << 4;
    fa[ks] = (wm * 64 + r32) * 128 + sw;
    fb[ks] = 16384 + (wn * 64 + r32) * 128 + sw;
  }
  const uint4 *msrc;
  const int mdst = I8P_STAGE + (wave & 3) * 1024;
  const int fm0 = I8P_STAGE + (wm * 64 + r32) * 32 + h * 16;

  i32x16 accg[2][2], accm[2][2];
#pragma unroll
  for (int i = 0; i < 2; ++i)
#pragma unroll
    for (int j = 0; j < 2; ++j)
#pragma unroll
      for (int r = 0; r < 16; ++r) { accg[i][j][r] = 0; accm[i][j][r] = 0; }

  i32x4 xa[2], xg[2], xb[2], ya[2], yg[2], yb[2], ms[2];
  unsigned mi[2];
  uint4 mc[2];
  const i32x4 mask_g = {0x03030303, 0x03030303, 0x03030303, 0x03030303};

#define SP_DMA(j, SOFF)                                                                                           \
  do {                                                                                                            \
    __builtin_amdgcn_global_load_lds((gemma_gptr_t)src[j], (gemma_lptr_t)(i8lds + (SOFF) + dst[j]), 16, 0, 0);    \
    src[j] += I8_BK;                                                                                              \
  } while (0)
#define SP_DMA_META(SOFF)                                                                                         \
  do {                                                                                                            \
    __builtin_amdgcn_global_load_lds((gemma_gptr_t)msrc, (gemma_lptr_t)(i8lds + (SOFF) + mdst), 16, 0, 0);        \
    msrc += 2;                                                                                                    \
  } while (0)
#define SP_READ_META(SOFF)                                                                                        \
  do {                                                                                                            \
    mc[0] = *reinterpret_cast<const uint4 *>(i8lds + (SOFF) + fm0);                                               \
    mc[1] = *reinterpret_cast<const uint4 *>(i8lds + (SOFF) + fm0 + 1024);                                        \
  } while (0)
#define SP_READ(q, SOFF, KS, RA, RB)                                                                              \
  do {                                                                                                            \
    if ((q) < 2) RA[(q)&1] = *reinterpret_cast<const i32x4 *>(i8lds + (SOFF) + fa[KS] + ((q)&1) * 4096);         \
    else RB[(q)&1] = *reinterpret_cast<const i32x4 *>(i8lds + (SOFF) + fb[KS] + ((q)&1) * 4096);                  \
  } while (0)
#define SP_MASK(i, RA, RG) RG[i] = RA[i] & mask_g
#define SP_G(b, RG, RB)                                                                                           \
  accg[(b) >> 1][(b)&1] = __builtin_amdgcn_mfma_i32_32x32x32_i8(RG[(b) >> 1], RB[(b)&1], accg[(b) >> 1][(b)&1], 0, 0, 0)
#define SP_S(b, PB, CB)                                                                                           \
  accm[(b) >> 1][(b)&1] = __builtin_amdgcn_smfmac_i32_32x32x64_i8(                                                \
      ms[(b) >> 1], __builtin_shufflevector(PB[(b)&1], CB[(b)&1], 0, 1, 2, 3, 4, 5, 6, 7), accm[(b) >> 1][(b)&1],  \
      (int)mi[(b) >> 1], 0, 0)
#define SP_OPER(P)                                                                                                \
  do {                                                                                                            \
    _Pragma("unroll") for (int i_ = 0; i_ < 2; ++i_) {                                                            \
      mi[i_] = (P) ? mc[i_].z : mc[i_].x;                                                                         \
      ms[i_] = sp_expand((P) ? mc[i_].w : mc[i_].y);                                                              \
    }                                                                                                             \
  } while (0)
#define SP_STEP_EVEN(CG, CB, NS, NKS, NA, NG, NB, DMA, D0, DS, META)                                              \
  do {                                                                                                            \
    SP_G(0, CG, CB); SP_READ(2, NS, NKS, NA, NB); GEMMA_SB();                                                     \
    SP_READ(3, NS, NKS, NA, NB); if (DMA) SP_DMA((D0) + 0, DS); GEMMA_SB();                                       \
    SP_G(1, CG, CB); SP_READ(0, NS, NKS, NA, NB); GEMMA_SB();                                                     \
    SP_READ(1, NS, NKS, NA, NB); if (DMA) SP_DMA((D0) + 1, DS); GEMMA_SB();                                       \
    SP_G(2, CG, CB); if (DMA) SP_DMA((D0) + 2, DS);                                                               \
    if (META) SP_DMA_META(DS);                                                                                    \
    GEMMA_SB();                                                                                                   \
    SP_G(3, CG, CB); SP_MASK(0, NA, NG); SP_MASK(1, NA, NG); GEMMA_SB();                                          \
  } while (0)
#define SP_STEP_ODD(CG, CB, PB, NS, NKS, NA, NG, NB, DMA, D0, DS)                                                 \
  do {                                                                                                            \
    SP_S(0, PB, CB); SP_READ(0, NS, NKS, NA, NB); GEMMA_SB();  \
    SP_S(1, PB, CB); SP_READ(1, NS, NKS, NA, NB); GEMMA_SB();                                                     \
    SP_S(2, PB, CB); if (DMA) SP_DMA((D0) + 0, DS); GEMMA_SB();                                                   \
    SP_S(3, PB, CB); if (DMA) SP_DMA((D0) + 1, DS); GEMMA_SB();                                                   \
    SP_G(0, CG, CB); SP_READ(2, NS, NKS, NA, NB); GEMMA_SB();                                                     \
    SP_G(1, CG, CB); SP_READ(3, NS, NKS, NA, NB); GEMMA_SB();                                                     \
    SP_G(2, CG, CB); if (DMA) SP_DMA((D0) + 2, DS); SP_MASK(0, NA, NG); GEMMA_SB();                               \
    SP_G(3, CG, CB); SP_MASK(1, NA, NG); GEMMA_SB();                                                              \
  } while (0)
#define SP_KTILE(SC, SN, SD, MORE, LOAD2)                                                                         \
  do {                                                                                                            \
    SP_OPER(0);                                                                                                   \
    SP_STEP_EVEN(xg, xb, SC, 1, ya, yg, yb, LOAD2, 0, SD, false);                                                 \
    SP_STEP_ODD(yg, yb, xb, SC, 2, xa, xg, xb, LOAD2, 3, SD);                                                     \
    SP_OPER(1);                                                                                                   \
    SP_STEP_EVEN(xg, xb, SC, 3, ya, yg, yb, false, 0, SD, LOAD2);                                                 \
    SP_S(0, xb, yb); GEMMA_SB();                                                                                  \
    SP_S(1, xb, yb); GEMMA_SB();                                                                                  \
    SP_S(2, xb, yb); GEMMA_SB();                                                                                  \
    SP_S(3, xb, yb); GEMMA_SB();                                                                                  \
    SP_G(0, yg, yb); GEMMA_SB();                                                                                  \
                     \
    if (LOAD2) asm volatile("s_waitcnt vmcnt(7)" ::: "memory");                                                   \
    else asm volatile("s_waitcnt vmcnt(0)" ::: "memory");                                                         \
    __builtin_amdgcn_s_barrier();                                                                                 \
    GEMMA_SB();                                                                                                   \
    SP_G(1, yg, yb); if (MORE) { SP_READ(0, SN, 0, xa, xb); SP_READ(1, SN, 0, xa, xb); } GEMMA_SB();              \
    SP_G(2, yg, yb); if (MORE) { SP_READ(2, SN, 0, xa, xb); SP_READ(3, SN, 0, xa, xb); } GEMMA_SB();              \
    SP_G(3, yg, yb); GEMMA_SB();                                                                                  \
    if (MORE) {                                                                                                   \
      SP_READ_META(SN);                                                                                           \
      SP_MASK(0, xa, xg); SP_MASK(1, xa, xg);                                                                     \
    }                                                                                                             \
  } while (0)

  const int nk = g.nk;
  for (int dd = 0; dd < nd; ++dd) {
    if (dd > 0) {
#pragma unroll
      for (int i = 0; i < 2; ++i)
#pragma unroll
        for (int j = 0; j < 2; ++j)
#pragma unroll
          for (int r = 0; r < 16; ++r) { accg[i][j][r] <<= 8; accm[i][j][r] <<= 8; }
    }
    SP_INIT_SRC(d_first - dd);
    msrc = sm.m4 + (((long)tm * I8P_BM + 32 * (wave & 3) + (lane >> 1)) * sm.ntiles) * 2 + (lane & 1);
#pragma unroll
    for (int j = 0; j < 6; ++j) SP_DMA(j, 0);
    SP_DMA_META(0);
    if (nk > 1) {
#pragma unroll
      for (int j = 0; j < 6; ++j) SP_DMA(j, SP_STAGE);
      SP_DMA_META(SP_STAGE);
      asm volatile("s_waitcnt vmcnt(7)" ::: "memory");
    } else {
      asm volatile("s_waitcnt vmcnt(0)" ::: "memory");
    }
    __builtin_amdgcn_s_barrier();
    GEMMA_SB();
#pragma unroll
    for (int q = 0; q < 4; ++q) SP_READ(q, 0, 0, xa, xb);
    SP_READ_META(0);
    SP_MASK(0, xa, xg);
    SP_MASK(1, xa, xg);

    int sc = 0, sn = SP_STAGE, sd = 2 * SP_STAGE;
    int kt = 0;
    for (; kt + 2 < nk; ++kt) {
      SP_KTILE(sc, sn, sd, true, true);
      const int tmp = sc; sc = sn; sn = sd; sd = tmp;
    }
    if (nk >= 2) {
      SP_KTILE(sc, sn, sd, true, false);
      const int tmp = sc; sc = sn; sn = sd; sd = tmp;
    }
    SP_KTILE(sc, sn, sd, false, false);
  }
#undef SP_INIT_SRC
#undef SP_DMA
#undef SP_READ
#undef SP_DMA_META
#undef SP_READ_META
#undef SP_MASK
#undef SP_G
#undef SP_S
#undef SP_OPER
#undef SP_STEP_EVEN
#undef SP_STEP_ODD
#undef SP_KTILE

  int *Cg = g.C + (long)plane * g.strideC;
#pragma unroll
  for (int i = 0; i < 2; ++i)
#pragma unroll
    for (int j = 0; j < 2; ++j) {
      const long col = (long)tn * I8_BN + wn * 64 + j * 32 + r32;
#pragma unroll
      for (int r = 0; r < 16; ++r) {
        const long row = (long)tm * I8P_BM + wm * 64 + i * 32 + (r & 3) + 8 * (r >> 2) + 4 * h;
        Cg[row * g.ldc + col] = accg[i][j][r];
        Cg[(g.m_row0 + row) * g.ldc + col] = accm[i][j][r];
      }
    }
}

}
```

### gemma_amd/csrc/i8gemm_sparse2.hip.h

```cpp
#pragma once
#include <algorithm>
#include <vector>
#include "i8gemm_sparse.hip.h"

namespace gemma_hip {

constexpr int S2_BM = 256, S2_BN = 128;
constexpr int S2_AMB = 16384;
constexpr int S2_STAGE = 32768;
constexpr int S2_NST = 4;
#ifndef S2_ADVANCE
#define S2_ADVANCE 1
#endif
#ifndef S2_LOOPDMA
#define S2_LOOPDMA 1
#endif

struct Sparse2Args {
  const uint4 *AM;
  const int8_t *Bt;
  int *C;
  long ldk, ldc, strideB, strideC, m_row0;
  int tiles_m, tiles_n, nk, gm, fuse, digits;
  int plane0 = 0;
  const int2 *tile_map = nullptr;
  const int *anymiss = nullptr;
  int run_if = 0;
  double *UtX = nullptr;
  long ldx = 0, l = 0, n = 0;
  const double *mean = nullptr, *qinv = nullptr;
  double m_scale = 1.0;
  int nplanes = 0;
};

__global__ __launch_bounds__(256) void sparse2_meta_kernel(const int8_t *__restrict__ A, long lpad, long ldk,
                                                           uint4 *__restrict__ AM, int *__restrict__ row_surplus,
                                                           int *anymiss = nullptr ) {
  const long nk = ldk / I8_BK;
  const long id = (long)blockIdx.x * 256 + threadIdx.x;
  if (id >= lpad * nk * 4) return;
  const int c = (int)(id & 3);
  const long rr = (id >> 2) & 255, tk = id >> 10;
  const long tmi = tk / nk, kt = tk - tmi * nk;
  const long row = tmi * S2_BM + rr;
  const int p = c >> 1, h = c & 1;
  const int8_t *base = A + row * ldk + kt * I8_BK;
  unsigned w[4];
#pragma unroll
  for (int e = 0; e < 2; ++e) {
    const int8_t *src = base + 32 * (2 * p + e) + 16 * h;
    unsigned g2 = 0;
#pragma unroll
    for (int i = 0; i < 4; ++i) g2 |= (*reinterpret_cast<const unsigned *>(src + 4 * i) & 0x03030303u) << (2 * i);
    w[e] = g2;
  }
  {
    const int8_t *src = base + 32 * (2 * p + h);
    unsigned idx = 0, bits = 0;
    int surplus = 0;
    for (int gq = 0; gq < 8; ++gq) {
      const unsigned word = *reinterpret_cast<const unsigned *>(src + 4 * gq);
      const unsigned m = (word >> 4) & 0x01010101u;
      const unsigned pat = (m | (m >> 7) | (m >> 14) | (m >> 21)) & 0xFu;
      const int cnt = __popc(pat);
      const int p0 = cnt >= 1 ? __ffs(pat) - 1 : 0;
      const unsigned rest = pat & (pat - 1);
      const int p1 = cnt >= 2 ? __ffs(rest) - 1 : (p0 == 3 ? 2 : 3);
      idx |= (unsigned)(p0 | (p1 << 2)) << (4 * gq);
      const int e0 = 2 * gq, e1 = 2 * gq + 1;
      bits |= (unsigned)(cnt >= 1) << (8 * (e0 & 3) + (e0 >> 2));
      bits |= (unsigned)(cnt >= 2) << (8 * (e1 & 3) + (e1 >> 2));
      surplus += cnt > 2 ? cnt - 2 : 0;
    }
    w[2] = idx;
    w[3] = bits;
    if (surplus) atomicAdd(row_surplus + row, surplus);
    if (anymiss && bits != 0 && *reinterpret_cast<volatile int *>(anymiss) == 0) *reinterpret_cast<volatile int *>(anymiss) = 1;
  }
  AM[id] = make_uint4(w[0], w[1], w[2], w[3]);
}

__device__ __forceinline__ i32x4 s2_unpack_g(int w) {
  i32x4 v;
  const unsigned u = (unsigned)w;
#pragma unroll
  for (int i = 0; i < 4; ++i) v[i] = (int)((u >> (2 * i)) & 0x03030303u);
  return v;
}
__device__ __forceinline__ i32x4 s2_expand(int bits) {
  i32x4 v;
  const unsigned u = (unsigned)bits;
#pragma unroll
  for (int i = 0; i < 4; ++i) v[i] = (int)((u >> i) & 0x01010101u);
  return v;
}

static inline void s2_build_raster(int tiles_m, int tiles_n, int rb, std::vector<int2> &map, int PR = 8) {
  const int NX = 8, PC = 32 / PR;
  if (rb != 1 && rb != 2 && rb != 4 && rb != 8) rb = 2;
  const int cbs = NX / rb;
  std::vector<std::vector<int2>> seq(NX);
  for (int band0 = 0, band = 0; band0 < tiles_m; band0 += rb * PR, ++band)
    for (int col0 = 0; col0 < tiles_n; col0 += cbs * PC)
      for (int xx = 0; xx < NX; ++xx) {
        const int x = (xx + band) % NX;
        const int r0 = band0 + (xx % rb) * PR, c0 = col0 + (xx / rb) * PC;
        const int nr = std::min(PR, std::min(tiles_m, band0 + rb * PR) - r0), nc = std::min(PC, std::min(tiles_n, col0 + cbs * PC) - c0);
        if (nr <= 0 || nc <= 0) continue;
        for (int c = 0; c < nc; ++c)
          for (int r = 0; r < nr; ++r) seq[x].push_back(make_int2(r0 + r, c0 + c));
      }
  const int total = tiles_m * tiles_n;
  std::vector<int> want(NX);
  for (int x = 0; x < NX; ++x) want[x] = total / NX + (x < total % NX ? 1 : 0);
  std::vector<int2> spare;
  for (int x = 0; x < NX; ++x)
    while ((int)seq[x].size() > want[x]) {
      spare.push_back(seq[x].back());
      seq[x].pop_back();
    }
  for (int x = 0; x < NX; ++x)
    while ((int)seq[x].size() < want[x]) {
      seq[x].push_back(spare.back());
      spare.pop_back();
    }
  map.assign((size_t)total, make_int2(0, 0));
  for (int x = 0; x < NX; ++x)
    for (int o = 0; o < want[x]; ++o) map[(size_t)o * NX + x] = seq[x][o];
}

template <int NI>
__global__ __launch_bounds__(512, 2) void i8gemm_sparse2_kernel_t(Sparse2Args g) {
  constexpr int NJ = 4 / NI;
  extern __shared__ __attribute__((aligned(1024))) int8_t i8lds[];
  int tm, tn;
  if (g.tile_map) {
    const int2 t2 = g.tile_map[blockIdx.x];
    tm = __builtin_amdgcn_readfirstlane(t2.x);
    tn = __builtin_amdgcn_readfirstlane(t2.y);
  } else {
    const int nwg = gridDim.x, b = blockIdx.x;
    const int q = nwg >> 3, r = nwg & 7, x = b & 7, o = b >> 3;
    const int L = (x < r ? x * (q + 1) : r * (q + 1) + (x - r) * q) + o;
    const int GM = g.gm > 0 ? g.gm : 8;
    const int per_group = GM * g.tiles_n;
    const int grp = L / per_group;
    const int first_m = grp * GM;
    const int gsz = min(g.tiles_m - first_m, GM);
    const int in = L - grp * per_group;
    tm = first_m + in % gsz;
    tn = in / gsz;
  }
  const int plane = blockIdx.y;
  const int odd = g.digits & 1;
  const int d_first = g.fuse ? (odd ? (plane == 0 ? 0 : 2 * plane) : 2 * plane + 1) : plane;
  const int nd = (g.fuse && !(odd && plane == 0)) ? 2 : 1;
  const int t = threadIdx.x, lane = t & 63;
  const int wave = __builtin_amdgcn_readfirstlane(t >> 6);
  const int wm = NI == 2 ? wave >> 1 : wave, wn = NI == 2 ? wave & 1 : 0;
  const int r32 = lane & 31, h = lane >> 5;

  const uint4 *asrc[2];
  const int8_t *bsrc[2];
  int adst[2], bdst[2];
#define S2_INIT_SRC(DIGIT)                                                                                        \
  do {                                                                                                            \
    _Pragma("unroll") for (int j = 0; j < 2; ++j) {                                                               \
      const int qp = 2 * wave + j;                                                                                \
      const int row = 16 * qp + (lane >> 2);                                                                      \
      asrc[j] = g.AM + ((long)tm * g.nk * S2_BM + row) * 4 + ((lane & 3) ^ ((row >> 2) & 3));                     \
      adst[j] = qp * 1024;                                                                                        \
      const int col = 8 * qp + (lane >> 3);                                                                       \
      bsrc[j] = g.Bt + (long)(DIGIT) * g.strideB + ((long)tn * S2_BN + col) * g.ldk + 16 * ((lane & 7) ^ ((col >> 1) & 7)); \
      bdst[j] = S2_AMB + qp * 1024;                                                                               \
    }                                                                                                             \
  } while (0)
  int amo[2], fb[4];
  {
    const int row = wm * 32 * NI + r32;
#pragma unroll
    for (int p = 0; p < 2; ++p) amo[p] = row * 64 + (((2 * p + h) ^ ((row >> 2) & 3)) << 4);
    const int col = wn * 32 * NJ + r32;
#pragma unroll
    for (int ks = 0; ks < 4; ++ks) fb[ks] = S2_AMB + col * 128 + (((2 * ks + h) ^ ((col >> 1) & 7)) << 4);
  }

  i32x16 accg[NI][NJ], accm[NI][NJ];
#pragma unroll
  for (int i = 0; i < NI; ++i)
#pragma unroll
    for (int j = 0; j < NJ; ++j)
#pragma unroll
      for (int r = 0; r < 16; ++r) { accg[i][j][r] = 0; accm[i][j][r] = 0; }

  i32x4 am[2][NI];
  i32x4 ga[2][NI];
  i32x4 bb[2][NJ];
  i32x4 ms[NI];

#define S2_DMA_A(j, SOFF)                                                                                         \
  do {                                                                                                            \
    __builtin_amdgcn_global_load_lds((gemma_gptr_t)asrc[j], (gemma_lptr_t)(i8lds + (SOFF) + adst[j]), 16, 0, 0);  \
    if (S2_ADVANCE) asrc[j] += S2_BM * 4;                                                                         \
  } while (0)
#define S2_DMA_B(j, SOFF)                                                                                         \
  do {                                                                                                            \
    __builtin_amdgcn_global_load_lds((gemma_gptr_t)bsrc[j], (gemma_lptr_t)(i8lds + (SOFF) + bdst[j]), 16, 0, 0);  \
    if (S2_ADVANCE) bsrc[j] += I8_BK;                                                                             \
  } while (0)
#define S2_RAM(SOFF, P, i) am[(P)&1][i] = *reinterpret_cast<const i32x4 *>(i8lds + (SOFF) + amo[(P)&1] + (i) * 2048)
#define S2_RB(SOFF, KS, j) bb[(KS)&1][j] = *reinterpret_cast<const i32x4 *>(i8lds + (SOFF) + fb[KS] + (j) * 4096)
#define S2_UNP(KS, i) ga[(KS)&1][i] = s2_unpack_g(am[((KS) >> 1) & 1][i][(KS)&1])
#define S2_EXP(P, i) ms[i] = s2_expand(am[(P)&1][i][3])
#define S2_G(KS, i, j)                                                                                            \
  asm volatile("s_nop 1\n\tv_mfma_i32_32x32x32_i8 %0, %1, %2, %0"                                                 \
               : "+v"(accg[i][j]) : "v"(ga[(KS)&1][i]), "v"(bb[(KS)&1][j]))
#define S2_S(P, i, j)                                                                                             \
  do {                                                                                                            \
    const i32x8 bp_ = __builtin_shufflevector(bb[0][j], bb[1][j], 0, 1, 2, 3, 4, 5, 6, 7);                         \
    asm volatile("s_nop 1\n\tv_smfmac_i32_32x32x64_i8 %0, %1, %2, %3"                                             \
                 : "+v"(accm[i][j]) : "v"(ms[i]), "v"(bp_), "v"(am[(P)&1][i][2]));                                 \
  } while (0)
#define S2_KTILE(SC, SN, SD, MORE, LOAD3, VMW)                                                                    \
  do {                                                                                                            \
         \
    S2_G(0, 0, 0); S2_RB(SC, 1, 0); GEMMA_SB();                                                                   \
    S2_G(0, 0, 1); S2_RB(SC, 1, 1); S2_EXP(0, 0); GEMMA_SB();                                                     \
    S2_G(0, 1, 0); if ((LOAD3) && S2_LOOPDMA) S2_DMA_A(0, SD); GEMMA_SB();                                                        \
    S2_G(0, 1, 1); S2_EXP(0, 1); GEMMA_SB();                                                                      \
         \
    S2_S(0, 0, 0); S2_RAM(SC, 1, 0); GEMMA_SB();                                                                  \
    S2_S(0, 0, 1); S2_RAM(SC, 1, 1); S2_UNP(1, 0); GEMMA_SB();                                                    \
    S2_S(0, 1, 0); if ((LOAD3) && S2_LOOPDMA) S2_DMA_A(1, SD); GEMMA_SB();                                                        \
    S2_S(0, 1, 1); S2_UNP(1, 1); GEMMA_SB();                                                                      \
        \
    S2_G(1, 0, 0); S2_UNP(2, 0); GEMMA_SB(); S2_RB(SC, 2, 0); GEMMA_SB();                                         \
    S2_G(1, 0, 1); S2_RB(SC, 2, 1); GEMMA_SB();                                                                   \
    S2_G(1, 1, 0); S2_UNP(2, 1); if ((LOAD3) && S2_LOOPDMA) S2_DMA_B(0, SD); GEMMA_SB();                                          \
    S2_G(1, 1, 1); if ((LOAD3) && S2_LOOPDMA) S2_DMA_B(1, SD); GEMMA_SB();                                                        \
     \
                                                     \
    S2_G(2, 0, 0); S2_RB(SC, 3, 0); GEMMA_SB();                                                                   \
    S2_G(2, 0, 1); S2_RB(SC, 3, 1); GEMMA_SB();                                                                   \
    asm volatile("s_waitcnt vmcnt(" #VMW ")" ::: "memory");                                                       \
    __builtin_amdgcn_s_barrier();                                                                                 \
    GEMMA_SB();                                                                                                   \
    S2_G(2, 1, 0); S2_EXP(1, 0); GEMMA_SB();                                                                      \
    S2_G(2, 1, 1); S2_EXP(1, 1); GEMMA_SB();                                                                      \
     \
    S2_S(1, 0, 0); if (MORE) S2_RAM(SN, 0, 0); GEMMA_SB();                                                        \
    S2_S(1, 0, 1); if (MORE) S2_RAM(SN, 0, 1); GEMMA_SB();                                                        \
    S2_S(1, 1, 0); S2_UNP(3, 0); GEMMA_SB();                                                                      \
    S2_S(1, 1, 1); S2_UNP(3, 1); GEMMA_SB();                                                                      \
     \
    S2_G(3, 0, 0); if (MORE) S2_UNP(0, 0); GEMMA_SB();                                                            \
    if (MORE) { S2_RB(SN, 0, 0); S2_RB(SN, 0, 1); } GEMMA_SB();                                                   \
    S2_G(3, 0, 1); if (MORE) S2_UNP(0, 1); GEMMA_SB();                                                            \
    S2_G(3, 1, 0); GEMMA_SB();                                                                                    \
    S2_G(3, 1, 1); GEMMA_SB();                                                                                    \
  } while (0)

#define S2_KTILE_81(SC, SN, SD, MORE, LOAD3, VMW)                                                                 \
  do {                                                                                                            \
    S2_G(0, 0, 0); S2_RB(SC, 1, 0); S2_RB(SC, 1, 1); GEMMA_SB();                                                  \
    S2_G(0, 0, 1); S2_RB(SC, 1, 2); S2_RB(SC, 1, 3); GEMMA_SB();                                                  \
    S2_G(0, 0, 2); S2_EXP(0, 0); if ((LOAD3) && S2_LOOPDMA) S2_DMA_A(0, SD); GEMMA_SB();                          \
    S2_G(0, 0, 3); GEMMA_SB();                                                                                    \
    S2_S(0, 0, 0); S2_RAM(SC, 1, 0); GEMMA_SB();                                                                  \
    S2_S(0, 0, 1); S2_UNP(1, 0); GEMMA_SB();                                                                      \
    S2_S(0, 0, 2); if ((LOAD3) && S2_LOOPDMA) S2_DMA_A(1, SD); GEMMA_SB();                                        \
    S2_S(0, 0, 3); GEMMA_SB();                                                                                    \
    S2_G(1, 0, 0); S2_UNP(2, 0); GEMMA_SB(); S2_RB(SC, 2, 0); S2_RB(SC, 2, 1); GEMMA_SB();                        \
    S2_G(1, 0, 1); S2_RB(SC, 2, 2); S2_RB(SC, 2, 3); GEMMA_SB();                                                  \
    S2_G(1, 0, 2); if ((LOAD3) && S2_LOOPDMA) S2_DMA_B(0, SD); GEMMA_SB();                                        \
    S2_G(1, 0, 3); if ((LOAD3) && S2_LOOPDMA) S2_DMA_B(1, SD); GEMMA_SB();                                        \
    S2_G(2, 0, 0); S2_RB(SC, 3, 0); S2_RB(SC, 3, 1); GEMMA_SB();                                                  \
    S2_G(2, 0, 1); S2_RB(SC, 3, 2); S2_RB(SC, 3, 3); GEMMA_SB();                                                  \
    asm volatile("s_waitcnt vmcnt(" #VMW ")" ::: "memory");                                                       \
    __builtin_amdgcn_s_barrier();                                                                                 \
    GEMMA_SB();                                                                                                   \
    S2_G(2, 0, 2); S2_EXP(1, 0); GEMMA_SB();                                                                      \
    S2_G(2, 0, 3); GEMMA_SB();                                                                                    \
    S2_S(1, 0, 0); if (MORE) S2_RAM(SN, 0, 0); GEMMA_SB();                                                        \
    S2_S(1, 0, 1); S2_UNP(3, 0); GEMMA_SB();                                                                      \
    S2_S(1, 0, 2); GEMMA_SB();                                                                                    \
    S2_S(1, 0, 3); GEMMA_SB();                                                                                    \
    S2_G(3, 0, 0); if (MORE) S2_UNP(0, 0); GEMMA_SB();                                                            \
    if (MORE) { S2_RB(SN, 0, 0); S2_RB(SN, 0, 1); } GEMMA_SB();                                                   \
    S2_G(3, 0, 1); if (MORE) { S2_RB(SN, 0, 2); S2_RB(SN, 0, 3); } GEMMA_SB();                                    \
    S2_G(3, 0, 2); GEMMA_SB();                                                                                    \
    S2_G(3, 0, 3); GEMMA_SB();                                                                                    \
  } while (0)
#define S2_TILE(SC, SN, SD, MORE, LOAD3, VMW)                                                                     \
  do {                                                                                                            \
    if constexpr (NI == 2) S2_KTILE(SC, SN, SD, MORE, LOAD3, VMW);                                                \
    else S2_KTILE_81(SC, SN, SD, MORE, LOAD3, VMW);                                                               \
  } while (0)
  if (wave >= 4) __builtin_amdgcn_s_setprio(1);
  const int nk = g.nk;
  for (int dd = 0; dd < nd; ++dd) {
    if (dd > 0) {
      asm volatile("s_nop 15\n\ts_nop 7" ::: "memory");
#pragma unroll
      for (int i = 0; i < NI; ++i)
#pragma unroll
        for (int j = 0; j < NJ; ++j)
#pragma unroll
          for (int r = 0; r < 16; ++r) { accg[i][j][r] <<= 8; accm[i][j][r] <<= 8; }
    }
    S2_INIT_SRC(d_first - dd);
#pragma unroll
    for (int j = 0; j < 2; ++j) { S2_DMA_A(j, 0); S2_DMA_B(j, 0); }
    if (nk > 1) {
#pragma unroll
      for (int j = 0; j < 2; ++j) { S2_DMA_A(j, S2_STAGE); S2_DMA_B(j, S2_STAGE); }
    }
    if (nk > 2) {
#pragma unroll
      for (int j = 0; j < 2; ++j) { S2_DMA_A(j, 2 * S2_STAGE); S2_DMA_B(j, 2 * S2_STAGE); }
      asm volatile("s_waitcnt vmcnt(8)" ::: "memory");
    } else if (nk > 1) {
      asm volatile("s_waitcnt vmcnt(4)" ::: "memory");
    } else {
      asm volatile("s_waitcnt vmcnt(0)" ::: "memory");
    }
    __builtin_amdgcn_s_barrier();
    GEMMA_SB();
#pragma unroll
    for (int i = 0; i < NI; ++i) S2_RAM(0, 0, i);
#pragma unroll
    for (int j = 0; j < NJ; ++j) S2_RB(0, 0, j);
#pragma unroll
    for (int i = 0; i < NI; ++i) S2_UNP(0, i);
    GEMMA_SB();

    int sc = 0, sn = S2_STAGE, s2 = 2 * S2_STAGE, sd = 3 * S2_STAGE;
    int kt = 0;
    for (; kt + 3 < nk; ++kt) {
      S2_TILE(sc, sn, sd, true, true, 8);
      const int tmp = sc; sc = sn; sn = s2; s2 = sd; sd = tmp;
    }
    if (nk >= 3) {
      S2_TILE(sc, sn, sd, true, false, 4);
      const int tmp = sc; sc = sn; sn = s2; s2 = sd; sd = tmp;
    }
    if (nk >= 2) {
      S2_TILE(sc, sn, sd, true, false, 0);
      const int tmp = sc; sc = sn; sn = s2; s2 = sd; sd = tmp;
    }
    S2_TILE(sc, sn, sd, false, false, 0);
  }
#undef S2_INIT_SRC
#undef S2_DMA_A
#undef S2_DMA_B
#undef S2_RAM
#undef S2_RB
#undef S2_UNP
#undef S2_EXP
#undef S2_G
#undef S2_S
#undef S2_KTILE
#undef S2_KTILE_81
#undef S2_TILE

  asm volatile("s_nop 15\n\ts_nop 7" ::: "memory");
  int *Cg = g.C + (long)plane * g.strideC;
#pragma unroll
  for (int i = 0; i < NI; ++i)
#pragma unroll
    for (int j = 0; j < NJ; ++j) {
      const long col = (long)tn * S2_BN + wn * 32 * NJ + j * 32 + r32;
#pragma unroll
      for (int r = 0; r < 16; ++r) {
        const long row = (long)tm * S2_BM + wm * 32 * NI + i * 32 + (r & 3) + 8 * (r >> 2) + 4 * h;
        Cg[row * g.ldc + col] = accg[i][j][r];
        Cg[(g.m_row0 + row) * g.ldc + col] = accm[i][j][r];
      }
    }
}

#ifndef S2_DEFAULT_RASTER
#define S2_DEFAULT_RASTER 1
#endif
#ifndef S2_DEFAULT_NI
#define S2_DEFAULT_NI 1
#endif
static constexpr auto i8gemm_sparse2_kernel = i8gemm_sparse2_kernel_t<S2_DEFAULT_NI>;

}
```

### gemma_amd/csrc/i8gemm_sparse2_r16.hip.h

```cpp
#pragma once
#include "i8gemm_sparse2.hip.h"

#ifndef S2_R16_PREP_SPREAD
#define S2_R16_PREP_SPREAD 0
#endif
#ifndef S2_R16_NST
#define S2_R16_NST 4
#endif
#ifndef S2_R16_ABL_NO_S
#define S2_R16_ABL_NO_S 0
#endif
#ifndef S2_R16_ABL_NO_D
#define S2_R16_ABL_NO_D 0
#endif

namespace gemma_hip {

constexpr int S2_R16_LDS = S2_R16_NST * S2_STAGE;

template <bool WITH_S, bool COMBINE = false>
__device__ __forceinline__ void s2_r16_body(const Sparse2Args &g) {
  extern __shared__ __attribute__((aligned(1024))) int8_t i8lds[];
  constexpr bool NO_S = !WITH_S || S2_R16_ABL_NO_S;
  if (g.run_if) {
    const int any = __builtin_amdgcn_readfirstlane(*g.anymiss);
    if ((g.run_if == 1) != (any != 0)) return;
  }
  int tm, tn;
  if (g.tile_map) {
    const int2 t2 = g.tile_map[blockIdx.x];
    tm = __builtin_amdgcn_readfirstlane(t2.x);
    tn = __builtin_amdgcn_readfirstlane(t2.y);
  } else {
    const int nwg = gridDim.x, b = blockIdx.x;
    const int q_ = nwg >> 3, r = nwg & 7, x = b & 7, o = b >> 3;
    const int L = (x < r ? x * (q_ + 1) : r * (q_ + 1) + (x - r) * q_) + o;
    const int GM = g.gm > 0 ? g.gm : 8;
    const int per_group = GM * g.tiles_n;
    const int grp = L / per_group;
    const int first_m = grp * GM;
    const int gsz = min(g.tiles_m - first_m, GM);
    const int in = L - grp * per_group;
    tm = first_m + in % gsz;
    tn = in / gsz;
  }
  const int plane = blockIdx.y + g.plane0;
  const int odd = g.digits & 1;
  const int d_first = g.fuse ? (odd ? (plane == 0 ? 0 : 2 * plane) : 2 * plane + 1) : plane;
  const int nd = (g.fuse && !(odd && plane == 0)) ? 2 : 1;
  const int t = threadIdx.x, lane = t & 63;
  const int wave = __builtin_amdgcn_readfirstlane(t >> 6);
  const int r16 = lane & 15, q = lane >> 4;

  const uint4 *asrc[2];
  const int8_t *bsrc[2];
  int adst[2], bdst[2];
#define GS_INIT_SRC(DIGIT)                                                                                        \
  do {                                                                                                            \
    _Pragma("unroll") for (int j = 0; j < 2; ++j) {                                                               \
      const int qp = 2 * wave + j;                                                                                \
      const int row = 16 * qp + (lane >> 2);                                                                      \
      asrc[j] = g.AM + ((long)tm * g.nk * S2_BM + row) * 4 + ((lane & 3) ^ ((row >> 2) & 3));                     \
      adst[j] = qp * 1024;                                                                                        \
      const int col = 8 * qp + (lane >> 3);                                                                       \
      bsrc[j] = g.Bt + (long)(DIGIT) * g.strideB + ((long)tn * S2_BN + col) * g.ldk + 16 * ((lane & 7) ^ ((col >> 1) & 7)); \
      bdst[j] = S2_AMB + qp * 1024;                                                                               \
    }                                                                                                             \
  } while (0)
  int ro[2], fo[2];
  {
    const int row = wave * 32 + r16;
#pragma unroll
    for (int p = 0; p < 2; ++p) {
      ro[p] = row * 64 + (((2 * p + (q & 1)) ^ ((row >> 2) & 3)) << 4);
      fo[p] = S2_AMB + r16 * 128 + (((4 * p + q) ^ ((r16 >> 1) & 7)) << 4);
    }
  }

  i32x4 accg[2][8], accm[2][8];
#pragma unroll
  for (int i = 0; i < 2; ++i)
#pragma unroll
    for (int j = 0; j < 8; ++j) { accg[i][j] = (i32x4){0, 0, 0, 0}; accm[i][j] = (i32x4){0, 0, 0, 0}; }

  i32x4 rec[2][2];
  i32x4 ga[2][2];
  i32x4 ms[2];
  int ix[2];
  i32x8 T[4];

#define GS_DMA_A(j, SOFF)                                                                                         \
  do {                                                                                                            \
    __builtin_amdgcn_global_load_lds((gemma_gptr_t)asrc[j], (gemma_lptr_t)(i8lds + (SOFF) + adst[j]), 16, 0, 0);  \
    asrc[j] += S2_BM * 4;                                                                                         \
  } while (0)
#define GS_DMA_B(j, SOFF)                                                                                         \
  do {                                                                                                            \
    __builtin_amdgcn_global_load_lds((gemma_gptr_t)bsrc[j], (gemma_lptr_t)(i8lds + (SOFF) + bdst[j]), 16, 0, 0);  \
    bsrc[j] += I8_BK;                                                                                             \
  } while (0)
#define GS_RREC(SOFF, i, P) rec[i][P] = *reinterpret_cast<const i32x4 *>(i8lds + (SOFF) + ro[P] + (i) * 1024)
#define GS_RT(SOFF, SB, SL)                                                                                       \
  do {                                                                                                            \
    const i32x4 x_ = *reinterpret_cast<const i32x4 *>(i8lds + (SOFF) + fo[0] + (SB) * 2048);                      \
    const i32x4 y_ = *reinterpret_cast<const i32x4 *>(i8lds + (SOFF) + fo[1] + (SB) * 2048);                      \
    T[SL] = __builtin_shufflevector(x_, y_, 0, 1, 2, 3, 4, 5, 6, 7);                                              \
  } while (0)
#define GS_PREP(i)                                                                                                \
  do {                                                                                                            \
    ga[i][0] = s2_unpack_g((q >> 1) ? rec[i][0][1] : rec[i][0][0]);                                               \
    ga[i][1] = s2_unpack_g((q >> 1) ? rec[i][1][1] : rec[i][1][0]);                                               \
    ix[i] = (q >> 1) ? rec[i][1][2] : rec[i][0][2];                                                               \
    ms[i] = s2_expand((q >> 1) ? rec[i][1][3] : rec[i][0][3]);                                                    \
    asm volatile("" ::"v"(rec[i][0]), "v"(rec[i][1]));                                                            \
  } while (0)
#define GS_PREP_G(i, P) ga[i][P] = s2_unpack_g((q >> 1) ? rec[i][P][1] : rec[i][P][0])
#define GS_PREP_M(i)                                                                                              \
  do {                                                                                                            \
    ix[i] = (q >> 1) ? rec[i][1][2] : rec[i][0][2];                                                               \
    ms[i] = s2_expand((q >> 1) ? rec[i][1][3] : rec[i][0][3]);                                                    \
    asm volatile("" ::"v"(rec[i][0]), "v"(rec[i][1]));                                                            \
  } while (0)
#define GS_D(i, SB, P, SL)                                                                                        \
  do {                                                                                                            \
    if (!S2_R16_ABL_NO_D)                                                                                         \
      asm volatile("s_nop 1\n\tv_mfma_i32_16x16x64_i8 %0, %1, %2, %0"                                             \
                   : "+v"(accg[i][SB])                                                                            \
                   : "v"(ga[i][P]), "v"(__builtin_shufflevector(T[SL], T[SL], 4 * (P), 4 * (P) + 1, 4 * (P) + 2, 4 * (P) + 3))); \
  } while (0)
#define GS_S(i, SB, SL)                                                                                           \
  do {                                                                                                            \
    if (!NO_S)                                                                                                    \
      asm volatile("s_nop 1\n\tv_smfmac_i32_16x16x128_i8 %0, %1, %2, %3" : "+v"(accm[i][SB]) : "v"(ms[i]), "v"(T[SL]), "v"(ix[i])); \
  } while (0)
#define GS_STEP(SB, SL, X)                                                                                        \
  do {                                                                                                            \
    GS_D(0, SB, 0, SL); GEMMA_SB();                                                                               \
    GS_D(1, SB, 0, SL); X; GEMMA_SB();                                                                            \
    GS_D(0, SB, 1, SL); GEMMA_SB();                                                                               \
    GS_D(1, SB, 1, SL); GEMMA_SB();                                                                               \
    GS_S(0, SB, SL); GEMMA_SB();                                                                                  \
    GS_S(1, SB, SL); GEMMA_SB();                                                                                  \
  } while (0)
#define GS_KTILE(SC, SN, SD, MORE, LOAD3, VMW)                                                                    \
  do {                                                                                                            \
    GS_STEP(0, 0, { GS_RT(SC, 3, 3); if (LOAD3) GS_DMA_A(0, SD); });                                               \
    GS_STEP(1, 1, { GS_RT(SC, 4, 0); if (LOAD3) GS_DMA_A(1, SD); });                                               \
    GS_STEP(2, 2, { GS_RT(SC, 5, 1); if (LOAD3) GS_DMA_B(0, SD); });                                               \
    GS_STEP(3, 3, { GS_RT(SC, 6, 2); if (LOAD3) GS_DMA_B(1, SD); });                                               \
    GS_STEP(4, 0, { GS_RT(SC, 7, 3); });                                                                           \
    asm volatile("s_waitcnt vmcnt(" #VMW ")" ::: "memory");                                                       \
    __builtin_amdgcn_s_barrier();                                                                                 \
    GEMMA_SB();                                                                                                   \
    GS_STEP(5, 1, { if (MORE) { GS_RREC(SN, 0, 0); GS_RREC(SN, 0, 1); GS_RREC(SN, 1, 0); GS_RREC(SN, 1, 1);       \
                                GS_RT(SN, 0, 0); } });                                                             \
    GS_STEP(6, 2, { if (MORE) { GS_RT(SN, 1, 1); } });                                                             \
    if (S2_R16_PREP_SPREAD && (MORE)) {                                                                           \
      GS_D(0, 7, 0, 3); GEMMA_SB();                                                                               \
      GS_D(1, 7, 0, 3); { GS_RT(SN, 2, 2); GS_PREP_G(0, 0); } GEMMA_SB();                                          \
      GS_D(0, 7, 1, 3); { GS_PREP_G(1, 0); } GEMMA_SB();                                                           \
      GS_D(1, 7, 1, 3); { GS_PREP_G(0, 1); } GEMMA_SB();                                                           \
      GS_S(0, 7, 3); { GS_PREP_G(1, 1); } GEMMA_SB();                                                              \
      GS_S(1, 7, 3); { GS_PREP_M(0); } GEMMA_SB();                                                                 \
      { GS_PREP_M(1); } GEMMA_SB();                                                                                \
    } else {                                                                                                      \
      GS_STEP(7, 3, { if (MORE) { GS_RT(SN, 2, 2); } });                                                           \
      if (MORE) { GS_PREP(0); GS_PREP(1); }                                                                       \
      GEMMA_SB();                                                                                                 \
    }                                                                                                             \
  } while (0)

  if (wave >= 4) __builtin_amdgcn_s_setprio(1);
  const int nk = g.nk;
  for (int dd = 0; dd < nd; ++dd) {
    if (dd > 0) {
      asm volatile("s_nop 15\n\ts_nop 7" ::: "memory");
#pragma unroll
      for (int i = 0; i < 2; ++i)
#pragma unroll
        for (int j = 0; j < 8; ++j)
#pragma unroll
          for (int r = 0; r < 4; ++r) {
            accg[i][j][r] <<= 8;
            if (WITH_S) accm[i][j][r] <<= 8;
          }
    }
    GS_INIT_SRC(d_first - dd);
#pragma unroll
    for (int j = 0; j < 2; ++j) { GS_DMA_A(j, 0); GS_DMA_B(j, 0); }
    if (nk > 1) {
#pragma unroll
      for (int j = 0; j < 2; ++j) { GS_DMA_A(j, S2_STAGE); GS_DMA_B(j, S2_STAGE); }
    }
    if (nk > 2) {
#pragma unroll
      for (int j = 0; j < 2; ++j) { GS_DMA_A(j, 2 * S2_STAGE); GS_DMA_B(j, 2 * S2_STAGE); }
    }
    if (S2_R16_NST == 5 && nk > 3) {
#pragma unroll
      for (int j = 0; j < 2; ++j) { GS_DMA_A(j, 3 * S2_STAGE); GS_DMA_B(j, 3 * S2_STAGE); }
      asm volatile("s_waitcnt vmcnt(12)" ::: "memory");
    } else if (nk > 2) {
      asm volatile("s_waitcnt vmcnt(8)" ::: "memory");
    } else if (nk > 1) {
      asm volatile("s_waitcnt vmcnt(4)" ::: "memory");
    } else {
      asm volatile("s_waitcnt vmcnt(0)" ::: "memory");
    }
    __builtin_amdgcn_s_barrier();
    GEMMA_SB();
    GS_RT(0, 0, 0);
    GS_RT(0, 1, 1);
    GS_RT(0, 2, 2);
    GS_RREC(0, 0, 0); GS_RREC(0, 0, 1); GS_RREC(0, 1, 0); GS_RREC(0, 1, 1);
    GS_PREP(0);
    GS_PREP(1);
    GEMMA_SB();

    int sc = 0, sn = S2_STAGE, s2 = 2 * S2_STAGE, s3 = 3 * S2_STAGE, sd = (S2_R16_NST - 1) * S2_STAGE;
#define GS_ROTATE()                                                                                               \
  do {                                                                                                            \
    const int tmp = sc;                                                                                           \
    sc = sn; sn = s2;                                                                                             \
    if (S2_R16_NST == 5) { s2 = s3; s3 = sd; } else { s2 = sd; }                                                  \
    sd = tmp;                                                                                                     \
  } while (0)
    int kt = 0;
    if (S2_R16_NST == 5) {
      for (; kt + 4 < nk; ++kt) {
        GS_KTILE(sc, sn, sd, true, true, 12);
        GS_ROTATE();
      }
      if (nk >= 4) {
        GS_KTILE(sc, sn, sd, true, false, 8);
        GS_ROTATE();
      }
    } else {
      for (; kt + 3 < nk; ++kt) {
        GS_KTILE(sc, sn, sd, true, true, 8);
        GS_ROTATE();
      }
    }
    if (nk >= 3) {
      GS_KTILE(sc, sn, sd, true, false, 4);
      GS_ROTATE();
    }
    if (nk >= 2) {
      GS_KTILE(sc, sn, sd, true, false, 0);
      GS_ROTATE();
    }
    GS_KTILE(sc, sn, sd, false, false, 0);
#undef GS_ROTATE
  }

  asm volatile("s_nop 15\n\ts_nop 7" ::: "memory");
  if constexpr (COMBINE) {
    const int np = g.nplanes;
    const bool load_m = !(g.anymiss && __builtin_amdgcn_readfirstlane(*g.anymiss) == 0);
    const double w_hi = g.fuse ? 65536.0 : 256.0;
    const double w0 = (g.fuse && !odd) ? 65536.0 : 256.0;
    const long row_w = (long)tm * S2_BM + wave * 32, col_w = (long)tn * S2_BN;
    const long row_l = row_w + 4 * q, col_l = col_w + r16;
    const unsigned lo_c = (unsigned)((4 * q * g.ldc + r16) * 4), lo_x = (unsigned)((4 * q * g.ldx + r16) * 8);
#define EP_AT(T, BASE, LO) (*(T *)((const char *)(BASE) + (LO)))
#define EP_LOAD(DG, DM, I, H, P)                                                                                  \
  do {                                                                                                            \
    const int *cp_ = g.C + (long)(P) * g.strideC + (row_w + 16 * (I)) * g.ldc + col_w + 32 * (H);                 \
    _Pragma("unroll") for (int k_ = 0; k_ < 2; ++k_) _Pragma("unroll") for (int r_ = 0; r_ < 4; ++r_) {           \
      DG[4 * k_ + r_] = EP_AT(const int, cp_ + r_ * g.ldc + 16 * k_, lo_c);                                       \
      DM[4 * k_ + r_] = load_m ? EP_AT(const int, cp_ + (g.m_row0 + r_) * g.ldc + 16 * k_, lo_c) : 0;             \
    }                                                                                                             \
  } while (0)
    int cg[8], cm[8];
#pragma unroll
    for (int e = 0; e < 8; ++e) cg[e] = cm[e] = 0;
    if (np > 1) EP_LOAD(cg, cm, 0, 0, np - 1);
#pragma unroll
    for (int b = 0; b < 8; ++b) {
      const int i = b >> 2, h = b & 3;
      double tg[8], tk[8];
#pragma unroll
      for (int e = 0; e < 8; ++e) tg[e] = tk[e] = 0.0;
      for (int p = np - 1; p >= 1; --p) {
        int ng[8], nm[8];
#pragma unroll
        for (int e = 0; e < 8; ++e) ng[e] = nm[e] = 0;
        if (p > 1) EP_LOAD(ng, nm, i, h, p - 1);
        else if (b < 7) EP_LOAD(ng, nm, (b + 1) >> 2, (b + 1) & 3, np - 1);
#pragma unroll
        for (int e = 0; e < 8; ++e) {
          tg[e] = tg[e] * w_hi + (double)cg[e];
          tk[e] = tk[e] * w_hi + (double)cm[e];
          cg[e] = ng[e];
          cm[e] = nm[e];
        }
      }
#pragma unroll
      for (int r = 0; r < 4; ++r) {
        const bool row_in = row_l + 16 * i + r < g.l;
        const double ms = row_in ? EP_AT(const double, g.mean + row_w + 16 * i + r, (unsigned)(32 * q)) * g.m_scale : 0.0;
#pragma unroll
        for (int k = 0; k < 2; ++k) {
          const int e = 4 * k + r, sb = 2 * h + k;
          const int m0 = WITH_S ? accm[i][sb][r] : 0;
          tg[e] = tg[e] * w0 + (double)accg[i][sb][r];
          tk[e] = tk[e] * w0 + (double)m0;
          if (row_in && col_l + 16 * sb < g.n)
            EP_AT(double, g.UtX + (row_w + 16 * i + r) * g.ldx + col_w + 16 * sb, lo_x) =
                fma(ms, tk[e], tg[e]) * EP_AT(const double, g.qinv + col_w + 16 * sb, (unsigned)(8 * r16));
        }
      }
    }
#undef EP_AT
#undef EP_LOAD
  } else {
    int *Cg = g.C + (long)plane * g.strideC;
#pragma unroll
    for (int i = 0; i < 2; ++i)
#pragma unroll
      for (int sb = 0; sb < 8; ++sb) {
        const long col = (long)tn * S2_BN + 16 * sb + r16;
#pragma unroll
        for (int r = 0; r < 4; ++r) {
          const long row = (long)tm * S2_BM + wave * 32 + 16 * i + 4 * q + r;
          Cg[row * g.ldc + col] = accg[i][sb][r];
          if (WITH_S) Cg[(g.m_row0 + row) * g.ldc + col] = accm[i][sb][r];
        }
      }
  }
#undef GS_INIT_SRC
#undef GS_DMA_A
#undef GS_DMA_B
#undef GS_RREC
#undef GS_RT
#undef GS_PREP
#undef GS_PREP_G
#undef GS_PREP_M
#undef GS_D
#undef GS_S
#undef GS_STEP
#undef GS_KTILE
}

__global__ __launch_bounds__(512, 2) void i8gemm_sparse2_r16_kernel(Sparse2Args g) { s2_r16_body<true>(g); }
__global__ __launch_bounds__(512, 2) void i8gemm_sparse2_r16_g_kernel(Sparse2Args g) { s2_r16_body<false>(g); }
__global__ __launch_bounds__(512, 2) void i8gemm_sparse2_r16_ep_kernel(Sparse2Args g) { s2_r16_body<true, true>(g); }
__global__ __launch_bounds__(512, 2) void i8gemm_sparse2_r16_ep_g_kernel(Sparse2Args g) { s2_r16_body<false, true>(g); }

}
```

Baseline: 368,800.

## Build sparse int8 GEMM records directly from PLINK 2-bit rows and pipeline epilogue loads

Adds a kernel that decodes PLINK 2-bit genotype rows straight into the sparse-product metadata records, mean and surplus counts. This skips materialising the int8 byte matrix and running the separate metadata build pass. Surplus list and fix kernels are templated so they can read the pattern from either source. The combine epilogue also gains a fixed-plane-count path that parks mask accumulators in LDS and prefetches C planes several stages deep. The new paths add complexity and carry a risk of subtle decode mismatches.

```diff
diff --git a/gemma_amd/build.py b/gemma_amd/build.py
--- a/gemma_amd/build.py
+++ b/gemma_amd/build.py
@@ -6,7 +6,7 @@
 CSRC = os.path.join(HERE, "csrc")
 LIB = os.path.join(HERE, "libgemma_hip.so")
 UNITS = {
-    "gemma_hip.hip": ["dgemm_mfma.hip.h", "lmm_grid.hip.h", "lmm_score_panel.hip.h", "i8gemm.hip.h", "i8gemm_sparse.hip.h", "i8gemm_sparse2.hip.h", "i8gemm_sparse2_r16.hip.h", "i8gemm_dense16.hip.h", "lmm_assoc.hip.h",
+    "gemma_hip.hip": ["dgemm_mfma.hip.h", "lmm_grid.hip.h", "lmm_score_panel.hip.h", "i8gemm.hip.h", "i8gemm_sparse.hip.h", "i8gemm_sparse2.hip.h", "i8gemm_sparse2_r16.hip.h", "plink_records.hip.h", "i8gemm_dense16.hip.h", "lmm_assoc.hip.h",
                       "lmm_search.hip.h", "comm.hip.h", "comm_shm.hpp", "kin_i8.hip.h", "ingest.hip.h", "qc.hip.h", "lm_assoc.hip.h", "mvlmm.hip.h",
                       "mvlmm_kernels.hip.h", "eigh_tu.h", "tu_common.h",
                       "abi_kinship.inc.h", "abi_eigen_qc.inc.h", "abi_lmm_stage.inc.h", "abi_utx.inc.h", "abi_lmm_batch.inc.h",
diff --git a/gemma_amd/csrc/abi_lmm_batch.inc.h b/gemma_amd/csrc/abi_lmm_batch.inc.h
--- a/gemma_amd/csrc/abi_lmm_batch.inc.h
+++ b/gemma_amd/csrc/abi_lmm_batch.inc.h
@@ -172,18 +172,9 @@
   double *UtX = g_ctx.UtX.as<double>();
   g_ctx.last_utx_path = 1;
   I8Dims d;
-  if ((rc = i8_begin(l, &d, s))) return rc;
-  {
-    ProfScope ps(GEMMA_STAGE_INGEST, s);
-    IngestI8Args a;
-    a.src = reinterpret_cast<const unsigned char *>(geno); a.ld = (long)ld; a.l = (long)l;
-    a.idx_map = g_ctx.have_map ? g_ctx.idx_map.as<int>() : nullptr;
-    a.n = (int)d.n; a.A = g_ctx.i8_A.as<int8_t>(); a.ldk = (long)d.ldk;
-    a.mean = g_ctx.i8_mean.as<double>();
-    hipLaunchKernelGGL(ingest_i8_kernel, dim3((unsigned)((l + 3) / 4)), dim3(256), 0, s, a);
-    HIPCHK(hipGetLastError());
-  }
-  if ((rc = i8_meta_build(d, s))) return rc;
+  const bool direct = i8_plink_direct();
+  if ((rc = i8_begin(l, &d, s, true, !direct))) return rc;
+  if ((rc = i8_plink_left(geno, l, ld, d, s, direct))) return rc;
   const size_t per = round_up((l + chunks - 1) / chunks, (size_t)S2_BM);
   hipStream_t side = g_ctx.ov_stream;
   int c = 0;
@@ -237,19 +228,8 @@
   g_ctx.last_utx_path = 1;
   I8Dims d;
   if ((rc = i8_begin(l, &d, x.P, false))) return xp_abort(rc);
-  {
-    ProfScope ps(GEMMA_STAGE_INGEST, x.P);
-    IngestI8Args a;
-    a.src = reinterpret_cast<const unsigned char *>(geno); a.ld = (long)ld; a.l = (long)l;
-    a.idx_map = g_ctx.have_map ? g_ctx.idx_map.as<int>() : nullptr;
-    a.n = (int)d.n; a.A = g_ctx.i8_A.as<int8_t>(); a.ldk = (long)d.ldk;
-    a.mean = g_ctx.i8_mean.as<double>();
-    hipLaunchKernelGGL(ingest_i8_kernel, dim3((unsigned)((l + 3) / 4)), dim3(256), 0, x.P, a);
-    if (hipGetLastError() != hipSuccess) return xp_abort(fail(GEMMA_HIP_ERUNTIME, "lmm_batch_pipe: ingest launch"));
-  }
-  if (hipEventRecord(x.ingest_done, x.P) != hipSuccess) return xp_abort(fail(GEMMA_HIP_ERUNTIME, "lmm_batch_pipe: event"));
+  if ((rc = i8_plink_left(geno, l, ld, d, x.P, false, x.ingest_done))) return xp_abort(rc);
   x.ingest_valid = true;
-  if ((rc = i8_meta_build(d, x.P))) return xp_abort(rc);
   if ((rc = i8_gemm_rows(d, 0, d.lpad, x.P))) return xp_abort(rc);
   HIPCHK(hipEventRecord(x.prod_done[slot], x.P));
   HIPCHK(hipStreamWaitEvent(x.Q, x.prod_done[slot], 0));
diff --git a/gemma_amd/csrc/abi_utx.inc.h b/gemma_amd/csrc/abi_utx.inc.h
--- a/gemma_amd/csrc/abi_utx.inc.h
+++ b/gemma_amd/csrc/abi_utx.inc.h
@@ -4,11 +4,13 @@
   int fuse, digits, nplanes;
   int mdrop;
   int complete;
+  const unsigned char *bed = nullptr;
+  long bed_ld = 0;
   int epi;
 };
 static const int *i8_anymiss(const I8Dims &d) { return d.complete ? g_ctx.i8_rowsur.as<int>() + d.lpad : nullptr; }
 static int i8_sparse_mode() { return g_ctx.knobs.i8_sparse; }
-static int i8_begin(size_t l, I8Dims *d, hipStream_t s, bool allow_epi = true) {
+static int i8_begin(size_t l, I8Dims *d, hipStream_t s, bool allow_epi = true, bool with_bytes = true) {
   int rc = i8_prepare_u(s);
   if (rc) return rc;
   d->n = g_ctx.cfg.n; d->ldk = g_ctx.i8_ldk; d->npad = g_ctx.i8_npad;
@@ -20,9 +22,10 @@
   d->complete = (g_ctx.knobs.i8_complete && i8_sparse_mode() == 2 && g_ctx.knobs.i8_rows == 16) ? 1 : 0;
   d->epi = (allow_epi && g_ctx.knobs.i8_epilogue && i8_sparse_mode() == 2 && g_ctx.knobs.i8_rows == 16 && d->nplanes >= 2) ? 1 : 0;
   const size_t c_elems = (size_t)(d->nplanes - d->epi) * d->mrows * d->npad;
-  if (g_ctx.i8_A.reserve(d->lpad * d->ldk) || g_ctx.i8_C.reserve(c_elems * 4) || g_ctx.i8_mean.reserve(l * 8))
-    return fail(GEMMA_HIP_ENOMEM, "lmm_batch: int8 product buffers (%zu bytes)", d->lpad * d->ldk + c_elems * 4);
-  if (d->lpad != l) HIPCHK(hipMemsetAsync(g_ctx.i8_A.p, 0, d->lpad * d->ldk, s));
+  const size_t a_bytes = with_bytes ? d->lpad * d->ldk : 0;
+  if ((with_bytes && g_ctx.i8_A.reserve(a_bytes)) || g_ctx.i8_C.reserve(c_elems * 4) || g_ctx.i8_mean.reserve(l * 8))
+    return fail(GEMMA_HIP_ENOMEM, "lmm_batch: int8 product buffers (%zu bytes)", a_bytes + c_elems * 4);
+  if (with_bytes && d->lpad != l) HIPCHK(hipMemsetAsync(g_ctx.i8_A.as<int8_t>() + l * d->ldk, 0, (d->lpad - l) * d->ldk, s));
   return GEMMA_HIP_OK;
 }
 
@@ -147,7 +150,7 @@
       g2.plane0 = 0;
       g2.UtX = UtX + row0 * ldx; g2.ldx = (long)ldx; g2.l = (long)rows; g2.n = (long)d.n;
       g2.mean = g_ctx.i8_mean.as<double>() + row0; g2.qinv = g_ctx.i8_qinv.as<double>();
-      g2.m_scale = 1.0; g2.nplanes = d.nplanes;
+      g2.m_scale = 1.0; g2.nplanes = d.nplanes; g2.epi_depth = g_ctx.knobs.i8_epi_depth;
       if (d.mdrop) {
         g2.run_if = 0;
         hipLaunchKernelGGL(i8gemm_sparse2_r16_ep_g_kernel, dim3(wgs, 1u), dim3(512), S2_R16_LDS, s, g2);
@@ -199,14 +202,19 @@
   const bool sparse = i8_sparse_mode() != 0;
   ProfScope ps(GEMMA_STAGE_UTX_POST, s);
   int *sur_cnt = nullptr, *sur_list = nullptr;
-  const int8_t *Arow = g_ctx.i8_A.as<int8_t>() + row0 * d.ldk;
+  const SurplusBytes from_bytes{g_ctx.i8_A.as<int8_t>() + row0 * d.ldk, (long)d.ldk};
+  const SurplusPlink from_bed{d.bed ? d.bed + row0 * d.bed_ld : nullptr, d.bed_ld, (long)d.n};
   if (sparse) {
     if (g_ctx.i8_surlist.reserve(l * (SUR_MAX + 1) * sizeof(int)))
       return fail(GEMMA_HIP_ENOMEM, "lmm_batch: dropped-call lists");
     sur_cnt = g_ctx.i8_surlist.as<int>() + row0;
     sur_list = g_ctx.i8_surlist.as<int>() + l + row0 * SUR_MAX;
-    hipLaunchKernelGGL(i8_surplus_list_kernel, dim3((unsigned)((rows + 3) / 4)), dim3(256), 0, s, Arow, (long)d.ldk,
-                       g_ctx.i8_rowsur.as<int>() + row0, (long)rows, sur_cnt, sur_list);
+    if (d.bed)
+      hipLaunchKernelGGL(i8_surplus_list_kernel<SurplusPlink>, dim3((unsigned)((rows + 3) / 4)), dim3(256), 0, s, from_bed,
+                         (long)d.ldk, g_ctx.i8_rowsur.as<int>() + row0, (long)rows, sur_cnt, sur_list);
+    else
+      hipLaunchKernelGGL(i8_surplus_list_kernel<SurplusBytes>, dim3((unsigned)((rows + 3) / 4)), dim3(256), 0, s, from_bytes,
+                         (long)d.ldk, g_ctx.i8_rowsur.as<int>() + row0, (long)rows, sur_cnt, sur_list);
     HIPCHK(hipGetLastError());
   }
   if (!d.epi) {
@@ -222,9 +230,14 @@
     HIPCHK(hipGetLastError());
   }
   if (sparse) {
-    hipLaunchKernelGGL(i8_surplus_fix_kernel, dim3((unsigned)rows), dim3(256), 0, s, Arow, (long)d.ldk,
-                       g_ctx.i8_rowsur.as<int>() + row0, g_ctx.i8_mean.as<double>() + row0, g_ctx.U, (long)d.n, (long)d.n,
-                       (long)rows, UtX + row0 * ldx, (long)ldx, SUR_MAX);
+    if (d.bed)
+      hipLaunchKernelGGL(i8_surplus_fix_kernel<SurplusPlink>, dim3((unsigned)rows), dim3(256), 0, s, from_bed, (long)d.ldk,
+                         g_ctx.i8_rowsur.as<int>() + row0, g_ctx.i8_mean.as<double>() + row0, g_ctx.U, (long)d.n, (long)d.n,
+                         (long)rows, UtX + row0 * ldx, (long)ldx, SUR_MAX);
+    else
+      hipLaunchKernelGGL(i8_surplus_fix_kernel<SurplusBytes>, dim3((unsigned)rows), dim3(256), 0, s, from_bytes, (long)d.ldk,
+                         g_ctx.i8_rowsur.as<int>() + row0, g_ctx.i8_mean.as<double>() + row0, g_ctx.U, (long)d.n, (long)d.n,
+                         (long)rows, UtX + row0 * ldx, (long)ldx, SUR_MAX);
     HIPCHK(hipGetLastError());
   }
   return GEMMA_HIP_OK;
@@ -237,21 +250,52 @@
   return rc;
 }
 
+static bool i8_plink_direct() { return g_ctx.knobs.i8_direct && i8_sparse_mode() == 2 && !g_ctx.have_map; }
+
+static int i8_plink_left(const void *geno, size_t l, size_t ld, I8Dims &d, hipStream_t s, bool direct,
+                         hipEvent_t after_ingest = nullptr) {
+  if (!direct) {
+    {
+      ProfScope ps(GEMMA_STAGE_INGEST, s);
+      IngestI8Args a;
+      a.src = reinterpret_cast<const unsigned char *>(geno); a.ld = (long)ld; a.l = (long)l;
+      a.idx_map = g_ctx.have_map ? g_ctx.idx_map.as<int>() : nullptr;
+      a.n = (int)d.n; a.A = g_ctx.i8_A.as<int8_t>(); a.ldk = (long)d.ldk;
+      a.mean = g_ctx.i8_mean.as<double>();
+      hipLaunchKernelGGL(ingest_i8_kernel, dim3((unsigned)((l + 3) / 4)), dim3(256), 0, s, a);
+      HIPCHK(hipGetLastError());
+    }
+    if (after_ingest) HIPCHK(hipEventRecord(after_ingest, s));
+    return i8_meta_build(d, s);
+  }
+  if (after_ingest || i8_sparse_mode() != 2 || g_ctx.have_map)
+    return fail(GEMMA_HIP_ESTATE, "lmm_batch: records straight from the 2-bit rows on a path that needs the byte matrix");
+  ProfScope ps(GEMMA_STAGE_INGEST, s);
+  const size_t nk = d.ldk / I8_BK;
+  if (g_ctx.i8_meta.reserve(d.lpad * nk * 4 * sizeof(uint4)) || g_ctx.i8_rowsur.reserve((d.lpad + 1) * sizeof(int)))
+    return fail(GEMMA_HIP_ENOMEM, "lmm_batch: records of the sparse product");
+  HIPCHK(hipMemsetAsync(g_ctx.i8_rowsur.as<int>() + d.lpad, 0, sizeof(int), s));
+  PlinkRecordsArgs a;
+  a.src = reinterpret_cast<const unsigned char *>(geno); a.ld = (long)ld; a.l = (long)l; a.lpad = (long)d.lpad;
+  a.n = (int)d.n; a.ldk = (long)d.ldk;
+  a.AM = g_ctx.i8_meta.as<uint4>(); a.row_surplus = g_ctx.i8_rowsur.as<int>();
+  a.anymiss = const_cast<int *>(i8_anymiss(d)); a.mean = g_ctx.i8_mean.as<double>();
+  hipLaunchKernelGGL(plink_records_kernel, dim3((unsigned)(d.lpad / 4)), dim3(256), 0, s, a);
+  HIPCHK(hipGetLastError());
+  g_ctx.i8_flag_at = d.complete ? (long)d.lpad : -1;
+  g_ctx.i8_rowsur_n = (long)d.lpad;
+  d.bed = a.src; d.bed_ld = (long)ld;
+  return GEMMA_HIP_OK;
+}
+
 static int utx_plink_i8(const void *geno, size_t l, size_t ld, double *UtX, size_t ldx, hipStream_t s) {
   I8Dims d;
-  int rc = i8_begin(l, &d, s);
-  if (rc) return rc;
-  {
-    ProfScope ps(GEMMA_STAGE_INGEST, s);
-    IngestI8Args a;
-    a.src = reinterpret_cast<const unsigned char *>(geno); a.ld = (long)ld; a.l = (long)l;
-    a.idx_map = g_ctx.have_map ? g_ctx.idx_map.as<int>() : nullptr;
-    a.n = (int)d.n; a.A = g_ctx.i8_A.as<int8_t>(); a.ldk = (long)d.ldk;
-    a.mean = g_ctx.i8_mean.as<double>();
-    hipLaunchKernelGGL(ingest_i8_kernel, dim3((unsigned)((l + 3) / 4)), dim3(256), 0, s, a);
-    HIPCHK(hipGetLastError());
-  }
-  return i8_product(l, d, UtX, ldx, s);
+  const bool direct = i8_plink_direct();
+  int rc = i8_begin(l, &d, s, true, !direct);
+  if (!rc) rc = i8_plink_left(geno, l, ld, d, s, direct);
+  if (!rc) rc = i8_gemm_rows(d, 0, d.lpad, s, UtX, ldx, l);
+  if (!rc) rc = i8_post_rows(l, d, 0, l, UtX, ldx, s);
+  return rc;
 }
 
 static bool dosage_i8_enabled() { return g_ctx.knobs.dosage_i8 != 0; }
diff --git a/gemma_amd/csrc/gemma_hip.hip b/gemma_amd/csrc/gemma_hip.hip
--- a/gemma_amd/csrc/gemma_hip.hip
+++ b/gemma_amd/csrc/gemma_hip.hip
@@ -25,6 +25,7 @@
 #include "i8gemm_sparse.hip.h"
 #include "i8gemm_sparse2.hip.h"
 #include "i8gemm_sparse2_r16.hip.h"
+#include "plink_records.hip.h"
 #include "i8gemm_dense16.hip.h"
 #include "qc.hip.h"
 #include "mvlmm.hip.h"
@@ -53,6 +54,8 @@
   int i8_mdrop = 0;
   int i8_complete = 1;
   int i8_epilogue = 1;
+  int i8_epi_depth = 4;
+  int i8_direct = 1;
   int dosage_i8 = 1;
   int dosage_rows = 16;
   int overlap = 0;
@@ -90,6 +93,9 @@
     i8_complete = (ecp && ecp[0] == '0') ? 0 : 1;
     const char *eep = getenv("GEMMA_HIP_I8_EPILOGUE");
     i8_epilogue = (eep && eep[0] == '0') ? 0 : 1;
+    i8_epi_depth = geti("GEMMA_HIP_I8_EPI_DEPTH", 4) <= 1 ? 1 : 4;
+    const char *edr = getenv("GEMMA_HIP_I8_DIRECT");
+    i8_direct = (edr && edr[0] == '0') ? 0 : 1;
     const char *ed = getenv("GEMMA_HIP_UTX_DOSAGE_I8");
     dosage_i8 = (ed && ed[0] == '0') ? 0 : 1;
     dosage_rows = geti("GEMMA_HIP_DOSAGE_ROWS", 16) == 32 ? 32 : 16;
diff --git a/gemma_amd/csrc/i8gemm_sparse.hip.h b/gemma_amd/csrc/i8gemm_sparse.hip.h
--- a/gemma_amd/csrc/i8gemm_sparse.hip.h
+++ b/gemma_amd/csrc/i8gemm_sparse.hip.h
@@ -59,7 +59,30 @@
   return hipGetLastError() == hipSuccess ? 0 : 1;
 }
 
-__global__ __launch_bounds__(256) void i8_surplus_fix_kernel(const int8_t *__restrict__ A, long ldk,
+struct SurplusBytes {
+  const int8_t *A;
+  long ldk;
+  __device__ __forceinline__ unsigned pat(long s, long gq) const {
+    const unsigned word = *reinterpret_cast<const unsigned *>(A + s * ldk + 4 * gq);
+    const unsigned m = (word >> 4) & 0x01010101u;
+    return (m | (m >> 7) | (m >> 14) | (m >> 21)) & 0xFu;
+  }
+};
+struct SurplusPlink {
+  const unsigned char *src;
+  long ld, n;
+  __device__ __forceinline__ unsigned pat(long s, long gq) const {
+    const long left = n - 4 * gq;
+    if (left <= 0) return 0u;
+    const unsigned b = src[s * ld + gq];
+    const unsigned m = b & ~(b >> 1) & 0x55u;
+    const unsigned p = (m & 1u) | ((m >> 1) & 2u) | ((m >> 2) & 4u) | ((m >> 3) & 8u);
+    return left >= 4 ? p : p & ((1u << left) - 1u);
+  }
+};
+
+template <class Src>
+__global__ __launch_bounds__(256) void i8_surplus_fix_kernel(Src src, long ldk,
                                                              const int *__restrict__ row_surplus,
                                                              const double *__restrict__ mean, const double *__restrict__ U,
                                                              long ldu, long n, long l, double *__restrict__ UtX, long ldx,
@@ -74,9 +97,7 @@
     const long gq = g0 + t;
     int f0 = -1, f1 = -1;
     if (gq < ngroups) {
-      const unsigned word = *reinterpret_cast<const unsigned *>(A + s * ldk + 4 * gq);
-      const unsigned m = (word >> 4) & 0x01010101u;
-      unsigned pat = (m | (m >> 7) | (m >> 14) | (m >> 21)) & 0xFu;
+      unsigned pat = src.pat(s, gq);
       if (__popc(pat) > 2) {
         pat &= pat - 1;
         pat &= pat - 1;
@@ -108,7 +129,8 @@
 }
 
 static_assert(SUR_MAX >= 2, "SUR_MAX (i8gemm.hip.h) is the list stride of this kernel, of i8_combine_kernel and of the host's buffers");
-__global__ __launch_bounds__(256) void i8_surplus_list_kernel(const int8_t *__restrict__ A, long ldk, const int *__restrict__ row_surplus,
+template <class Src>
+__global__ __launch_bounds__(256) void i8_surplus_list_kernel(Src src, long ldk, const int *__restrict__ row_surplus,
                                                              long l, int *__restrict__ sur_cnt, int *__restrict__ sur_list) {
   const int lane = threadIdx.x & 63;
   const long s = (long)blockIdx.x * 4 + (threadIdx.x >> 6);
@@ -124,9 +146,7 @@
     const long gq = g0 + lane;
     int f0 = -1, f1 = -1;
     if (gq < ngroups) {
-      const unsigned word = *reinterpret_cast<const unsigned *>(A + s * ldk + 4 * gq);
-      const unsigned m = (word >> 4) & 0x01010101u;
-      unsigned pat = (m | (m >> 7) | (m >> 14) | (m >> 21)) & 0xFu;
+      unsigned pat = src.pat(s, gq);
       if (__popc(pat) > 2) {
         pat &= pat - 1;
         pat &= pat - 1;
diff --git a/gemma_amd/csrc/i8gemm_sparse2.hip.h b/gemma_amd/csrc/i8gemm_sparse2.hip.h
--- a/gemma_amd/csrc/i8gemm_sparse2.hip.h
+++ b/gemma_amd/csrc/i8gemm_sparse2.hip.h
@@ -31,6 +31,7 @@
   const double *mean = nullptr, *qinv = nullptr;
   double m_scale = 1.0;
   int nplanes = 0;
+  int epi_depth = 1;
 };
 
 __global__ __launch_bounds__(256) void sparse2_meta_kernel(const int8_t *__restrict__ A, long lpad, long ldk,
diff --git a/gemma_amd/csrc/i8gemm_sparse2_r16.hip.h b/gemma_amd/csrc/i8gemm_sparse2_r16.hip.h
--- a/gemma_amd/csrc/i8gemm_sparse2_r16.hip.h
+++ b/gemma_amd/csrc/i8gemm_sparse2_r16.hip.h
@@ -1,4 +1,5 @@
 #pragma once
+#include <type_traits>
 #include "i8gemm_sparse2.hip.h"
 
 #ifndef S2_R16_PREP_SPREAD
@@ -17,6 +18,7 @@
 namespace gemma_hip {
 
 constexpr int S2_R16_LDS = S2_R16_NST * S2_STAGE;
+static_assert(S2_R16_LDS >= 16 * 512 * 16, "the epilogue parks 16 x 16 bytes per lane of the mask accumulators in the launch's LDS");
 
 template <bool WITH_S, bool COMBINE = false>
 __device__ __forceinline__ void s2_r16_body(const Sparse2Args &g) {
@@ -271,6 +273,102 @@
       DM[4 * k_ + r_] = load_m ? EP_AT(const int, cp_ + (g.m_row0 + r_) * g.ldc + 16 * k_, lo_c) : 0;             \
     }                                                                                                             \
   } while (0)
+    constexpr int EP_DEPTH = 4;
+    if constexpr (WITH_S) {
+      __syncthreads();
+#pragma unroll
+      for (int j = 0; j < 16; ++j) *reinterpret_cast<i32x4 *>(i8lds + ((j * 512 + t) << 4)) = accm[j >> 3][j & 7];
+      GEMMA_SB();
+    }
+    typedef const __attribute__((address_space(1))) int *ep_gint_t;
+    typedef const __attribute__((address_space(1))) char *ep_gchar_t;
+#define EP_UNI(PTR)                                                                                               \
+  ((ep_gint_t)(((unsigned long)(unsigned)__builtin_amdgcn_readfirstlane((int)((unsigned long)(PTR) >> 32)) << 32) | \
+               (unsigned long)(unsigned)__builtin_amdgcn_readfirstlane((int)(unsigned long)(PTR))))
+#define EP_ATG(BASE, LO) (*(ep_gint_t)((ep_gchar_t)(BASE) + (LO)))
+#define EP_LOADF(DG, DM, I, H, P)                                                                                 \
+  do {                                                                                                            \
+    const int *cp_ = g.C + (long)(P) * g.strideC + (row_w + 16 * (I)) * g.ldc + col_w + 32 * (H);                 \
+    const ep_gint_t cg_ = EP_UNI(cp_), cm_ = EP_UNI(cp_ + g.m_row0 * g.ldc);                                      \
+    _Pragma("unroll") for (int k_ = 0; k_ < 2; ++k_) _Pragma("unroll") for (int r_ = 0; r_ < 4; ++r_) {           \
+      DG[4 * k_ + r_] = EP_ATG(cg_ + 16 * k_, lo_r[r_]);                                                          \
+      if constexpr (LM) DM[4 * k_ + r_] = EP_ATG(cm_ + 16 * k_, lo_r[r_]);                                        \
+      else DM[4 * k_ + r_] = 0;                                                                                   \
+    }                                                                                                             \
+  } while (0)
+    auto ep_fixed = [&](auto np_tag, auto lm_tag) {
+      constexpr int NP = decltype(np_tag)::value, SPB = NP - 1, NS = 8 * SPB;
+      constexpr bool LM = decltype(lm_tag)::value;
+      int qf = q, cf = r16;
+      asm volatile("" : "+v"(qf), "+v"(cf));
+      const long row_lf = row_w + 4 * qf, col_lf = col_w + cf;
+      const int rows_left = (int)min(g.l - row_lf, 64L), cols_left = (int)min(g.n - col_lf, 256L);
+      const unsigned lo_xf = (unsigned)((4 * qf * g.ldx + cf) * 8);
+      unsigned lo_r[4];
+#pragma unroll
+      for (int r = 0; r < 4; ++r) lo_r[r] = (unsigned)(((4 * qf + r) * g.ldc + cf) * 4);
+      double msv[2][4], qv[8];
+#pragma unroll
+      for (int i = 0; i < 2; ++i)
+#pragma unroll
+        for (int r = 0; r < 4; ++r)
+          msv[i][r] = g.mean[row_lf + min(16 * i + r, rows_left - 1)];
+#pragma unroll
+      for (int sb = 0; sb < 8; ++sb) qv[sb] = g.qinv[col_lf + min(16 * sb, cols_left - 1)];
+      GEMMA_SB();
+      int lg[EP_DEPTH][8], lm[EP_DEPTH][8];
+#pragma unroll
+      for (int s = 0; s < EP_DEPTH; ++s) {
+        EP_LOADF(lg[s], lm[s], (s / SPB) >> 2, (s / SPB) & 3, NP - 1 - s % SPB);
+        GEMMA_SB();
+      }
+#pragma unroll
+      for (int b = 0; b < 8; ++b) {
+        const int i = b >> 2, h = b & 3;
+        double tg[8], tk[8];
+#pragma unroll
+        for (int e = 0; e < 8; ++e) tg[e] = tk[e] = 0.0;
+#pragma unroll
+        for (int j = 0; j < SPB; ++j) {
+          const int s = SPB * b + j, sl = s % EP_DEPTH, s2 = s + EP_DEPTH;
+#pragma unroll
+          for (int e = 0; e < 8; ++e) {
+            tg[e] = tg[e] * w_hi + (double)lg[sl][e];
+            tk[e] = tk[e] * w_hi + (double)lm[sl][e];
+          }
+          GEMMA_SB();
+          if (s2 < NS) EP_LOADF(lg[sl], lm[sl], (s2 / SPB) >> 2, (s2 / SPB) & 3, NP - 1 - s2 % SPB);
+          GEMMA_SB();
+        }
+        i32x4 mk[2] = {(i32x4){0, 0, 0, 0}, (i32x4){0, 0, 0, 0}};
+        if constexpr (WITH_S) {
+#pragma unroll
+          for (int k = 0; k < 2; ++k) mk[k] = *reinterpret_cast<const i32x4 *>(i8lds + (((8 * i + 2 * h + k) * 512 + t) << 4));
+        }
+#pragma unroll
+        for (int r = 0; r < 4; ++r) {
+          const bool row_in = 16 * i + r < rows_left;
+          const double ms = msv[i][r] * g.m_scale;
+#pragma unroll
+          for (int k = 0; k < 2; ++k) {
+            const int e = 4 * k + r, sb = 2 * h + k;
+            tg[e] = tg[e] * w0 + (double)accg[i][sb][r];
+            tk[e] = tk[e] * w0 + (double)mk[k][r];
+            if (row_in && 16 * sb < cols_left)
+              EP_AT(double, g.UtX + (row_w + 16 * i + r) * g.ldx + col_w + 16 * sb, lo_xf) =
+                  fma(ms, tk[e], tg[e]) * qv[sb];
+          }
+        }
+        GEMMA_SB();
+      }
+    };
+    if (g.epi_depth > 1 && np == 3) {
+      if (load_m) ep_fixed(std::integral_constant<int, 3>(), std::true_type());
+      else ep_fixed(std::integral_constant<int, 3>(), std::false_type());
+    } else if (g.epi_depth > 1 && np == 4) {
+      if (load_m) ep_fixed(std::integral_constant<int, 4>(), std::true_type());
+      else ep_fixed(std::integral_constant<int, 4>(), std::false_type());
+    } else {
     int cg[8], cm[8];
 #pragma unroll
     for (int e = 0; e < 8; ++e) cg[e] = cm[e] = 0;
@@ -295,6 +393,11 @@
           cm[e] = nm[e];
         }
       }
+      i32x4 mk[2] = {(i32x4){0, 0, 0, 0}, (i32x4){0, 0, 0, 0}};
+      if constexpr (WITH_S) {
+#pragma unroll
+        for (int k = 0; k < 2; ++k) mk[k] = *reinterpret_cast<const i32x4 *>(i8lds + (((8 * i + 2 * h + k) * 512 + t) << 4));
+      }
 #pragma unroll
       for (int r = 0; r < 4; ++r) {
         const bool row_in = row_l + 16 * i + r < g.l;
@@ -302,7 +405,7 @@
 #pragma unroll
         for (int k = 0; k < 2; ++k) {
           const int e = 4 * k + r, sb = 2 * h + k;
-          const int m0 = WITH_S ? accm[i][sb][r] : 0;
+          const int m0 = mk[k][r];
           tg[e] = tg[e] * w0 + (double)accg[i][sb][r];
           tk[e] = tk[e] * w0 + (double)m0;
           if (row_in && col_l + 16 * sb < g.n)
@@ -311,8 +414,12 @@
         }
       }
     }
+    }
 #undef EP_AT
 #undef EP_LOAD
+#undef EP_LOADF
+#undef EP_UNI
+#undef EP_ATG
   } else {
     int *Cg = g.C + (long)plane * g.strideC;
 #pragma unroll
diff --git a/gemma_amd/csrc/plink_records.hip.h b/gemma_amd/csrc/plink_records.hip.h
--- /dev/null
+++ b/gemma_amd/csrc/plink_records.hip.h
@@ -0,0 +1,144 @@
+#pragma once
+#include <stdint.h>
+#if defined(__HIPCC__)
+#include "i8gemm_sparse2.hip.h"
+#define PR_HD __host__ __device__ __forceinline__
+#else
+#define PR_HD inline
+#endif
+
+namespace gemma_hip {
+
+PR_HD int pr_popc(unsigned v) {
+#if defined(__HIP_DEVICE_COMPILE__)
+  return __popc(v);
+#else
+  return __builtin_popcount(v);
+#endif
+}
+
+PR_HD void pr_decode(unsigned w, int nvalid, unsigned *val, unsigned *miss) {
+  const unsigned valid = nvalid >= 16 ? 0x55555555u : (nvalid <= 0 ? 0u : ((1u << (2 * nvalid)) - 1u) & 0x55555555u);
+  const unsigned lo = w & 0x55555555u, hi = (w >> 1) & 0x55555555u;
+  const unsigned one = hi & ~lo & valid, two = ~(lo | hi) & valid;
+  *val = one | (two << 1);
+  *miss = lo & ~hi & valid;
+}
+PR_HD int pr_valsum(unsigned val) { return pr_popc(val & 0x55555555u) + 2 * pr_popc(val & 0xAAAAAAAAu); }
+
+PR_HD unsigned pr_genoword(unsigned val) {
+  unsigned t = ((val >> 6) ^ val) & 0x00CC00CCu;
+  val ^= t ^ (t << 6);
+  t = ((val >> 12) ^ val) & 0x0000F0F0u;
+  val ^= t ^ (t << 12);
+  return val;
+}
+
+PR_HD int pr_maskword(unsigned m0, unsigned m1, unsigned *idx_out, unsigned *bits_out) {
+  const unsigned K = 0x01010101u;
+  unsigned idx = 0, bits = 0;
+  int surplus = 0;
+#if defined(__HIP_DEVICE_COMPILE__)
+#pragma unroll
+#endif
+  for (int j = 0; j < 2; ++j) {
+    const unsigned m = j ? m1 : m0;
+    const unsigned a = m & K, b = (m >> 2) & K, c = (m >> 4) & K, d = (m >> 6) & K;
+    const unsigned na = a ^ K, nb = b ^ K, nc = c ^ K;
+    const unsigned ab = a & b, axb = a ^ b, cd = c & d;
+    const unsigned p0b0 = na & (b | (nc & d)), p0b1 = na & nb & (c | d);
+    const unsigned s1 = ab, s2 = axb & c, s3 = d & (axb ^ c) & ((ab & c) ^ K);
+    const unsigned ge1 = a | b | c | d, ge2 = s1 | s2 | s3, nge2 = ge2 ^ K;
+    const unsigned only_d = d & na & nb & nc;
+    const unsigned p1b0 = s1 | s3 | (nge2 & (only_d ^ K)), p1b1 = s2 | s3 | nge2;
+    const unsigned nib = p0b0 | (p0b1 << 1) | (p1b0 << 2) | (p1b1 << 3);
+    idx |= ((nib & 0xFu) | ((nib >> 4) & 0xF0u) | ((nib >> 8) & 0xF00u) | ((nib >> 12) & 0xF000u)) << (16 * j);
+    const unsigned k1 = (ge1 & 1u) | ((ge1 >> 8) & 1u) << 16 | ((ge1 >> 16) & 1u) << 1 | ((ge1 >> 24) & 1u) << 17;
+    const unsigned k2 = (ge2 & 1u) | ((ge2 >> 8) & 1u) << 16 | ((ge2 >> 16) & 1u) << 1 | ((ge2 >> 24) & 1u) << 17;
+    bits |= (k1 | (k2 << 8)) << (2 * j);
+    surplus += pr_popc((ab & (c | d)) | (cd & (a | b))) + pr_popc(ab & cd);
+  }
+  *idx_out = idx;
+  *bits_out = bits;
+  return surplus;
+}
+
+template <class Word>
+PR_HD int pr_record(Word word, long kt, int c, long n, unsigned w[4], int *tot, int *miss) {
+  const int p = c >> 1, h = c & 1;
+  const long kb = 8 * kt + 4 * p;
+  const long ka = kb + h, kc = kb + 2 + h, km = kb + 1 + h;
+  const long ra = n - 16 * ka, rc = n - 16 * kc, rm = n - 16 * km;
+  unsigned va, vc, vm, ma, mc, mm;
+  pr_decode(ra > 0 ? word(ka) : 0u, (int)(ra < 16 ? ra : 16), &va, &ma);
+  pr_decode(rc > 0 ? word(kc) : 0u, (int)(rc < 16 ? rc : 16), &vc, &mc);
+  pr_decode(rm > 0 ? word(km) : 0u, (int)(rm < 16 ? rm : 16), &vm, &mm);
+  const unsigned m0 = h ? mm : ma, m1 = h ? mc : mm;
+  w[0] = pr_genoword(va);
+  w[1] = pr_genoword(vc);
+  *tot += pr_valsum(va) + pr_valsum(vc);
+  *miss += pr_popc(m0 | (m1 << 1));
+  return pr_maskword(m0, m1, &w[2], &w[3]);
+}
+
+#if defined(__HIPCC__)
+struct PlinkRecordsArgs {
+  const unsigned char *src;
+  long ld, l, lpad;
+  int n;
+  long ldk;
+  uint4 *AM;
+  int *row_surplus;
+  int *anymiss;
+  double *mean;
+};
+
+__device__ __forceinline__ unsigned pr_load(const unsigned char *bs, long k, long nbytes, bool aligned) {
+  const long o = 4 * k;
+  if (aligned && o + 4 <= nbytes) return *reinterpret_cast<const unsigned *>(bs + o);
+  unsigned w = 0u;
+#pragma unroll
+  for (int b = 0; b < 4; ++b)
+    if (o + b < nbytes) w |= (unsigned)bs[o + b] << (8 * b);
+  return w;
+}
+
+__global__ __launch_bounds__(256) void plink_records_kernel(PlinkRecordsArgs g) {
+  const int lane = threadIdx.x & 63;
+  const long row = (long)blockIdx.x * 4 + (threadIdx.x >> 6);
+  if (row >= g.lpad) return;
+  const long nk = g.ldk / I8_BK, items = nk * 4;
+  uint4 *out = g.AM + ((row / S2_BM) * nk * S2_BM + (row % S2_BM)) * 4;
+  if (row >= g.l) {
+    for (long id = lane; id < items; id += 64) out[(id >> 2) * (S2_BM * 4) + (id & 3)] = make_uint4(0u, 0u, 0xCCCCCCCCu, 0u);
+    if (lane == 0) g.row_surplus[row] = 0;
+    return;
+  }
+  const unsigned char *bs = g.src + row * g.ld;
+  const bool aligned = (reinterpret_cast<uintptr_t>(bs) & 3) == 0;
+  const long nbytes = ((long)g.n + 3) / 4;
+  int itot = 0, imiss = 0, isur = 0;
+  unsigned anybits = 0;
+  for (long id = lane; id < items; id += 64) {
+    const long kt = id >> 2;
+    const int c = (int)(id & 3);
+    unsigned w[4];
+    isur += pr_record([&](long k) { return pr_load(bs, k, nbytes, aligned); }, kt, c, (long)g.n, w, &itot, &imiss);
+    anybits |= w[3];
+    out[kt * (S2_BM * 4) + c] = make_uint4(w[0], w[1], w[2], w[3]);
+  }
+#pragma unroll
+  for (int o = 32; o > 0; o >>= 1) {
+    itot += __shfl_xor(itot, o, 64);
+    imiss += __shfl_xor(imiss, o, 64);
+    isur += __shfl_xor(isur, o, 64);
+  }
+  if (lane == 0) {
+    g.mean[row] = (double)itot / (double)(g.n - imiss);
+    g.row_surplus[row] = isur;
+  }
+  if (g.anymiss && anybits != 0 && *reinterpret_cast<volatile int *>(g.anymiss) == 0) *reinterpret_cast<volatile int *>(g.anymiss) = 1;
+}
+#endif
+
+}
```

After: 374,800 (median of 6 runs). 1.02x the previous value.
